# FaspDevTeam/faspsolver

Hardware: AMD Instinct MI355X
Metric: AMG-PCG solve DOF/s (3D 7-pt Poisson 256^3, classical AMG V(1,1) w-Jacobi + PCG, rtol 1e-8) (higher is better)
Workload: dtype f64

## Files before the change

faspsolver_amd/__init__.py:

```python
import ctypes as C
import os
import subprocess

import numpy as np

from . import _types as T
from ._types import *

_HERE = os.path.dirname(os.path.abspath(__file__))
LIB_PATH = os.environ.get("FASP_HIP_LIB") or os.path.join(_HERE, "libfasp_hip.so")
_lib = None

EXPORTS = [
    "fasp_param_amg_init", "fasp_param_solver_init", "fasp_solver_dcsr_krylov_amg",
    "fasp_blas_dcsr_mxv", "fasp_blas_dcsr_aAxpy", "fasp_blas_darray_dotprod",
    "fasp_blas_darray_norm2", "fasp_blas_darray_norminf", "fasp_blas_darray_axpy",
    "fasp_blas_darray_axpby", "fasp_smoother_dcsr_jacobi",
    "fasp_blas_dbsr_mxv", "fasp_blas_dbsr_aAxpy", "fasp_dbsr_getdiaginv", "fasp_smoother_dbsr_jacobi1",
    "fasp_solver_dbsr_pcg", "fasp_solver_dbsr_pbcgs", "fasp_solver_dbsr_pgmres", "fasp_solver_dbsr_pvgmres",
    "fasp_solver_dbsr_pvfgmres", "fasp_hip_bsr_precond_setup", "fasp_hip_bsr_precond_fct", "fasp_hip_bsr_precond_free",
    "fasp_hip_param_input", "fasp_fwrapper_dcsr_krylov_amg_", "fasp_dcsrvec_read2", "fasp_dvec_read",
    "fasp_dbsr_read", "fasp_dcoo_read", "fasp_dcoo_read1", "fasp_dcoo_shift_read", "fasp_dmtx_read", "fasp_dmtxsym_read", "fasp_dvec_write", "fasp_dcsr_write_coo", "fasp_dcsrvec_write2", "fasp_fwrapper_dcsr_amg_", "fasp_fwrapper_dbsr_krylov_amg_", "fasp_hip_free_bsr", "fasp_hip_comm_selftest", "fasp_hip_amg_kernel_info", "fasp_hip_coarse_kernel_info", "fasp_hip_bsr_coarse_kernel_info", "fasp_hip_coding_selftest", "fasp_solver_amg", "fasp_solver_famg", "fasp_hip_amg_solve", "fasp_precond_diag", "fasp_precond_dbsr_diag", "fasp_solver_dcsr_itsolver", "fasp_solver_dcsr_krylov", "fasp_solver_dcsr_krylov_diag", "fasp_solver_dbsr_itsolver", "fasp_solver_dbsr_krylov", "fasp_solver_dbsr_krylov_diag", "fasp_hip_mxv_csr", "fasp_hip_mxv_bsr", "fasp_solver_matfree_init", "fasp_solver_pcg", "fasp_solver_pbcgs", "fasp_solver_pgcg", "fasp_solver_pminres", "fasp_solver_pgmres", "fasp_solver_pvgmres", "fasp_solver_pvfgmres", "fasp_solver_itsolver", "fasp_solver_krylov", "fasp_solver_dcsr_pcg", "fasp_solver_dcsr_pminres", "fasp_solver_dcsr_pgcg", "fasp_solver_dcsr_pgcr", "fasp_solver_dcsr_pbcgs", "fasp_solver_dcsr_pgmres", "fasp_solver_dcsr_pvgmres",
    "fasp_solver_dcsr_pvfgmres", "fasp_hip_precond_setup", "fasp_hip_precond_fct", "fasp_hip_precond_free",
    "fasp_hip_time_bsr_mxv", "fasp_solver_dbsr_krylov_amg", "fasp_hip_bsr_amg_create", "fasp_hip_bsr_amg_create_host",
    "fasp_hip_bsr_amg_destroy", "fasp_hip_bsr_amg_num_levels", "fasp_hip_bsr_amg_get_matrix",
    "fasp_hip_bsr_amg_get_diaginv", "fasp_hip_bsr_solve",
    "fasp_hip_set_device", "fasp_hip_device_count", "fasp_hip_device_identity", "fasp_hip_available",
    "fasp_hip_amg_create", "fasp_hip_amg_create_host", "fasp_hip_amg_upload",
    "fasp_hip_amg_destroy", "fasp_hip_amg_num_levels", "fasp_hip_amg_get_matrix",
    "fasp_hip_amg_get_cfmark", "fasp_hip_solve", "fasp_hip_set_rhs", "fasp_hip_set_guess",
    "fasp_hip_solve_resident", "fasp_hip_get_solution", "fasp_hip_device_synchronize",
    "fasp_hip_precond_amg",
    "fasp_hip_poisson7pt", "fasp_hip_aniso27pt", "fasp_hip_free_system", "fasp_hip_time_kernel", "fasp_hip_measure_ceilings", "fasp_hip_amg_publish", "fasp_hip_amg_attach", "fasp_hip_amg_unpublish",
    "fasp_precond_setup", "fasp_precond_amg", "fasp_precond_famg", "fasp_precond_amli", "fasp_precond_namli", "fasp_amg_data_create", "fasp_amg_data_free", "fasp_param_amg_to_prec", "fasp_param_prec_to_amg", "fasp_mem_free", "fasp_mem_calloc", "fasp_dvec_alloc", "fasp_dvec_set", "fasp_dvec_free", "fasp_dvec_create", "fasp_dcsr_create", "fasp_dcsr_free", "fasp_smoother_dcsr_gs", "fasp_smoother_dcsr_sor", "fasp_smoother_dcsr_L1diag",
    "fasp_hip_tune", "fasp_hip_comm_unique_id", "fasp_hip_comm_init", "fasp_hip_comm_finalize",
    "fasp_hip_comm_rank", "fasp_hip_comm_size", "fasp_hip_version", "fasp_hip_comm_init_shm",
    "fasp_hip_dist_plan", "fasp_hip_dist_level_info", "fasp_hip_dist_get_matrix",
    "fasp_hip_dist_get_list",
    "fasp_blas_dcsr_vmv", "fasp_blas_dcsr_mxv_agg", "fasp_blas_dcsr_aAxpy_agg", "fasp_blas_darray_ax",
    "fasp_blas_darray_axpyz", "fasp_blas_darray_norm1", "fasp_darray_cp", "fasp_darray_set", "fasp_dvec_isnan",
    "fasp_hip_time_matrix", "fasp_hip_bsr_dist_info", "fasp_hip_seq_schedule_selftest", "fasp_hip_seq_chain_selftest", "fasp_hip_cluster_order", "fasp_hip_permute_csr", "fasp_hip_comm_init_ipc", "fasp_hip_comm_stats", "fasp_hip_comm_timing", "fasp_hip_estream_selftest", "fasp_hip_sell_selftest", "fasp_hip_csr_plan", "fasp_hip_level_op", "fasp_hip_matrix_op",
    "fasp_param_ilu_init", "fasp_ilu_data_create", "fasp_ilu_data_free", "fasp_mem_iludata_check", "fasp_ilu_dcsr_setup",
    "fasp_precond_ilu", "fasp_precond_ilu_forward", "fasp_precond_ilu_backward", "fasp_solver_dcsr_krylov_ilu",
    "fasp_solver_dcsr_krylov_ilu_M", "fasp_smoother_dcsr_ilu", "fasp_fwrapper_dcsr_krylov_ilu_",
    "fasp_hip_ilu_resident_count", "fasp_hip_ilu_time",
    "fasp_ilu_dbsr_setup", "fasp_precond_dbsr_ilu", "fasp_solver_dbsr_krylov_ilu", "fasp_smoother_dbsr_ilu",
    "fasp_fwrapper_dbsr_krylov_ilu_",
    "fasp_hip_bsr_amg_get_ilu", "fasp_hip_bsr_amg_ilu_info", "fasp_hip_bsr_amg_ilu_smooth_time",
    "fasp_hip_bsr_sweep",
    "fasp_blas_dcsr_rap", "fasp_hip_dcsr_rap", "fasp_hip_rap_info", "fasp_hip_rap_device_count", "fasp_hip_rap_time",
]


def build(verbose=False):
    cmd = ["make", "-C", os.path.join(_HERE, "csrc")]
    if not verbose:
        cmd.insert(1, "-s")
    subprocess.run(cmd, check=True)


def lib():
    global _lib
    if _lib is not None:
        return _lib
    if not os.path.exists(LIB_PATH):
        build()
    L = C.CDLL(LIB_PATH)
    P = C.POINTER
    L.fasp_param_amg_init.argtypes = [P(T.AMG_param)]
    L.fasp_param_solver_init.argtypes = [P(T.ITS_param)]
    L.fasp_solver_dcsr_krylov_amg.argtypes = [P(T.dCSRmat), P(T.dvector), P(T.dvector),
                                              P(T.ITS_param), P(T.AMG_param)]
    L.fasp_blas_dcsr_mxv.argtypes = [P(T.dCSRmat), T.c_double_p, T.c_double_p]
    L.fasp_blas_dcsr_aAxpy.argtypes = [C.c_double, P(T.dCSRmat), T.c_double_p, T.c_double_p]
    for f in ("fasp_blas_darray_dotprod", "fasp_blas_darray_norm2", "fasp_blas_darray_norminf"):
        getattr(L, f).restype = C.c_double
    L.fasp_blas_darray_dotprod.argtypes = [C.c_int, T.c_double_p, T.c_double_p]
    L.fasp_blas_darray_norm2.argtypes = [C.c_int, T.c_double_p]
    L.fasp_blas_darray_norminf.argtypes = [C.c_int, T.c_double_p]
    L.fasp_blas_darray_axpy.argtypes = [C.c_int, C.c_double, T.c_double_p, T.c_double_p]
    L.fasp_blas_darray_axpby.argtypes = [C.c_int, C.c_double, T.c_double_p, C.c_double,
                                         T.c_double_p]
    L.fasp_blas_dcsr_vmv.restype = C.c_double
    L.fasp_blas_dcsr_vmv.argtypes = [P(T.dCSRmat), T.c_double_p, T.c_double_p]
    L.fasp_blas_dcsr_mxv_agg.argtypes = [P(T.dCSRmat), T.c_double_p, T.c_double_p]
    L.fasp_blas_dcsr_aAxpy_agg.argtypes = [C.c_double, P(T.dCSRmat), T.c_double_p, T.c_double_p]
    L.fasp_blas_darray_ax.argtypes = [C.c_int, C.c_double, T.c_double_p]
    L.fasp_blas_darray_axpyz.argtypes = [C.c_int, C.c_double, T.c_double_p, T.c_double_p, T.c_double_p]
    L.fasp_blas_darray_norm1.restype = C.c_double
    L.fasp_blas_darray_norm1.argtypes = [C.c_int, T.c_double_p]
    L.fasp_darray_cp.argtypes = [C.c_int, T.c_double_p, T.c_double_p]
    L.fasp_darray_set.argtypes = [C.c_int, T.c_double_p, C.c_double]
    L.fasp_hip_time_matrix.restype = C.c_double
    L.fasp_hip_time_matrix.argtypes = [P(T.dCSRmat), C.c_int, C.c_int, P(C.c_int)]
    L.fasp_dvec_isnan.restype = C.c_short
    L.fasp_dvec_isnan.argtypes = [P(T.dvector)]
    L.fasp_smoother_dcsr_jacobi.argtypes = [P(T.dvector), C.c_int, C.c_int, C.c_int,
                                            P(T.dCSRmat), P(T.dvector), C.c_int, C.c_double]
    L.fasp_blas_dbsr_mxv.argtypes = [P(T.dBSRmat), T.c_double_p, T.c_double_p]
    L.fasp_blas_dbsr_aAxpy.argtypes = [C.c_double, P(T.dBSRmat), T.c_double_p, T.c_double_p]
    L.fasp_dbsr_getdiaginv.argtypes = [P(T.dBSRmat)]
    L.fasp_dbsr_getdiaginv.restype = T.dvector
    L.fasp_smoother_dbsr_jacobi1.argtypes = [P(T.dBSRmat), P(T.dvector), P(T.dvector), T.c_double_p]
    L.fasp_hip_bsr_sweep.argtypes = [P(T.dBSRmat), T.c_double_p, T.c_double_p, T.c_double_p, C.c_int, C.c_int, C.c_double,
                                     P(C.c_int)]
    L.fasp_hip_time_bsr_mxv.argtypes = [P(T.dBSRmat), C.c_int]
    L.fasp_hip_time_bsr_mxv.restype = C.c_double
    L.fasp_solver_dcsr_pcg.argtypes = [P(T.dCSRmat), P(T.dvector), P(T.dvector), P(T.precond), C.c_double,
                                       C.c_double, C.c_int, C.c_short, C.c_short]
    L.fasp_solver_dcsr_pbcgs.argtypes = L.fasp_solver_dcsr_pcg.argtypes
    L.fasp_solver_dcsr_pminres.argtypes = L.fasp_solver_dcsr_pcg.argtypes
    L.fasp_solver_dcsr_pgcg.argtypes = L.fasp_solver_dcsr_pcg.argtypes
    L.fasp_solver_dcsr_pvgmres.argtypes = [P(T.dCSRmat), P(T.dvector), P(T.dvector), P(T.precond), C.c_double,
                                           C.c_double, C.c_int, C.c_short, C.c_short, C.c_short]
    L.fasp_solver_dcsr_pvfgmres.argtypes = L.fasp_solver_dcsr_pvgmres.argtypes
    L.fasp_solver_dcsr_pgmres.argtypes = L.fasp_solver_dcsr_pvgmres.argtypes
    L.fasp_solver_dcsr_pgcr.argtypes = L.fasp_solver_dcsr_pvgmres.argtypes
    L.fasp_hip_precond_setup.argtypes = [P(T.dCSRmat), P(T.AMG_param)]
    L.fasp_hip_precond_setup.restype = P(T.precond)
    L.fasp_hip_precond_free.argtypes = [P(T.precond)]
    L.fasp_hip_precond_free.restype = None
    L.fasp_hip_precond_fct.argtypes = [T.c_double_p, T.c_double_p, C.c_void_p]
    L.fasp_hip_precond_fct.restype = None
    L.fasp_solver_dbsr_pcg.argtypes = [P(T.dBSRmat), P(T.dvector), P(T.dvector), P(T.precond), C.c_double,
                                       C.c_double, C.c_int, C.c_short, C.c_short]
    L.fasp_solver_dbsr_pbcgs.argtypes = L.fasp_solver_dbsr_pcg.argtypes
    L.fasp_solver_dbsr_pvgmres.argtypes = [P(T.dBSRmat), P(T.dvector), P(T.dvector), P(T.precond), C.c_double,
                                           C.c_double, C.c_int, C.c_short, C.c_short, C.c_short]
    L.fasp_solver_dbsr_pgmres.argtypes = L.fasp_solver_dbsr_pvgmres.argtypes
    L.fasp_solver_dbsr_pvfgmres.argtypes = L.fasp_solver_dbsr_pvgmres.argtypes
    L.fasp_hip_bsr_precond_setup.argtypes = [P(T.dBSRmat), P(T.AMG_param)]
    L.fasp_hip_bsr_precond_setup.restype = P(T.precond)
    L.fasp_hip_bsr_precond_free.argtypes = [P(T.precond)]
    L.fasp_hip_bsr_precond_free.restype = None
    L.fasp_hip_bsr_precond_fct.argtypes = [T.c_double_p, T.c_double_p, C.c_void_p]
    L.fasp_hip_bsr_precond_fct.restype = None
    L.fasp_dcsrvec_read2.argtypes = [C.c_char_p, C.c_char_p, P(T.dCSRmat), P(T.dvector)]
    L.fasp_dvec_read.argtypes = [C.c_char_p, P(T.dvector)]
    L.fasp_dbsr_read.argtypes = [C.c_char_p, P(T.dBSRmat)]
    L.fasp_hip_free_bsr.argtypes = [P(T.dBSRmat)]
    L.fasp_hip_free_bsr.restype = None
    L.fasp_hip_param_input.argtypes = [C.c_char_p, P(T.ITS_param), P(T.AMG_param)]
    L.fasp_fwrapper_dcsr_krylov_amg_.argtypes = [P(C.c_int), P(C.c_int), T.c_int_p, T.c_int_p, T.c_double_p,
                                                 T.c_double_p, T.c_double_p, P(C.c_double), P(C.c_int), P(C.c_int)]
    L.fasp_fwrapper_dcsr_krylov_amg_.restype = None
    L.fasp_hip_coding_selftest.argtypes = [P(T.dCSRmat), P(C.c_int)]
    L.fasp_hip_amg_kernel_info.argtypes = [C.c_void_p, C.c_int, C.c_int, P(C.c_int), P(C.c_double)]
    L.fasp_hip_coarse_kernel_info.argtypes = [C.c_void_p, P(C.c_int)]
    L.fasp_hip_bsr_coarse_kernel_info.argtypes = [C.c_void_p, P(C.c_int)]
    L.fasp_solver_amg.argtypes = [P(T.dCSRmat), P(T.dvector), P(T.dvector), P(T.AMG_param)]
    L.fasp_hip_amg_solve.argtypes = [C.c_void_p, P(T.dvector), P(T.dvector), P(T.AMG_param), T.c_double_p,
                                     C.c_int, P(T.fasp_hip_stats)]
    L.fasp_solver_dbsr_krylov_amg.argtypes = [P(T.dBSRmat), P(T.dvector), P(T.dvector), P(T.ITS_param),
                                              P(T.AMG_param)]
    L.fasp_hip_bsr_amg_create.argtypes = [P(C.c_void_p), P(T.dBSRmat), P(T.AMG_param)]
    L.fasp_hip_bsr_amg_create_host.argtypes = [P(C.c_void_p), P(T.dBSRmat), P(T.AMG_param)]
    L.fasp_hip_bsr_amg_destroy.argtypes = [C.c_void_p]
    L.fasp_hip_bsr_amg_destroy.restype = None
    L.fasp_hip_bsr_amg_num_levels.argtypes = [C.c_void_p]
    L.fasp_hip_bsr_amg_get_matrix.argtypes = [C.c_void_p, C.c_int, C.c_int, P(T.dBSRmat)]
    L.fasp_hip_bsr_amg_get_diaginv.argtypes = [C.c_void_p, C.c_int]
    L.fasp_hip_bsr_amg_get_diaginv.restype = T.c_double_p
    L.fasp_hip_bsr_solve.argtypes = [C.c_void_p, P(T.dvector), P(T.dvector), P(T.ITS_param), T.c_double_p,
                                     C.c_int, P(T.fasp_hip_stats)]
    L.fasp_hip_amg_create.argtypes = [P(C.c_void_p), P(T.dCSRmat), P(T.AMG_param)]
    L.fasp_hip_amg_create_host.argtypes = L.fasp_hip_amg_create.argtypes
    L.fasp_hip_amg_upload.argtypes = [C.c_void_p]
    L.fasp_hip_amg_destroy.argtypes = [C.c_void_p]
    L.fasp_hip_amg_destroy.restype = None
    L.fasp_hip_amg_num_levels.argtypes = [C.c_void_p]
    L.fasp_hip_amg_get_matrix.argtypes = [C.c_void_p, C.c_int, C.c_int, P(T.dCSRmat)]
    L.fasp_hip_amg_get_cfmark.argtypes = [C.c_void_p, C.c_int, P(T.ivector)]
    L.fasp_hip_solve.argtypes = [C.c_void_p, P(T.dvector), P(T.dvector), P(T.ITS_param),
                                 T.c_double_p, C.c_int, P(T.fasp_hip_stats)]
    L.fasp_hip_set_rhs.argtypes = [C.c_void_p, P(T.dvector)]
# ... 471 lines not shown
```

faspsolver_amd/csrc/coarse_cg.hip.h:

```cpp

static bool small_coarse_ok(long long rows, long long stored_values)
{
    static int enabled = -1;
    if (enabled < 0) {
        const char* e = std::getenv("FASP_HIP_SMALL_COARSE");
        enabled = (e && std::atoi(e) == 0) ? 0 : 1;
    }
    return enabled && rows <= 4096 && stored_values <= 131072;
}
static SmallOut* small_out_dev() { return reinterpret_cast<SmallOut*>(g_ctx.d_partials2); }
static int small_out_fetch(SmallOut& o)
{
    HIPCK(hipMemcpyAsync(g_ctx.h_part, g_ctx.d_partials2, sizeof(SmallOut), hipMemcpyDeviceToHost, g_ctx.stream));
    HIPCK(hipStreamSynchronize(g_ctx.stream));
    std::memcpy(&o, g_ctx.h_part, sizeof(SmallOut));
    return 0;
}

static bool g_persist_disabled = false;
static bool build_persist_plan(fasp_hip_amg* h, int level)
{
    auto& P = h->persist;
    if (P.tried) return P.ok;
    P.tried = true;
    const HostCSR& A = h->H.L[(size_t)level].A;
    const int m = A.row;
    const int nblocks = g_ctx.num_cu, nw = (nblocks - 1) * 8;
    if (m < 1 || m > 6144 || m != A.col || nw < 8 || A.nnz <= 0) return false;
    std::vector<int> order((size_t)m), slots((size_t)m);
    for (int i = 0; i < m; ++i) { order[(size_t)i] = i; slots[(size_t)i] = (A.ia[i + 1] - A.ia[i] + 63) / 64; }
    std::stable_sort(order.begin(), order.end(), [&](int x, int y) { return slots[(size_t)x] > slots[(size_t)y]; });
    std::vector<int> load((size_t)nw, 0), cnt((size_t)nw, 0), wrow((size_t)nw * 8, -1), wend((size_t)nw * 8, 0);
    std::vector<std::pair<int, int>> heap;
    for (int w = 0; w < nw; ++w) heap.emplace_back(0, w);
    auto cmp = [](const std::pair<int, int>& x, const std::pair<int, int>& y) { return x > y; };
    std::make_heap(heap.begin(), heap.end(), cmp);
    for (int i : order) {
        if (slots[(size_t)i] == 0) continue;
        std::pop_heap(heap.begin(), heap.end(), cmp);
        std::pair<int, int> top = heap.back();
        const int w = top.second;
        if (cnt[(size_t)w] >= 8) return false;
        load[(size_t)w] += slots[(size_t)i];
        wrow[(size_t)w * 8 + cnt[(size_t)w]] = i;
        wend[(size_t)w * 8 + cnt[(size_t)w]] = load[(size_t)w];
        cnt[(size_t)w]++;
        heap.back() = std::make_pair(load[(size_t)w], w);
        std::push_heap(heap.begin(), heap.end(), cmp);
    }
    for (int i = 0; i < m; ++i) if (slots[(size_t)i] == 0) return false;
    const int maxload = *std::max_element(load.begin(), load.end());
    const int NE = maxload <= 32 ? 32 : maxload <= 48 ? 48 : maxload <= 56 ? 56 : maxload <= 64 ? 64 : 0;
    if (!NE) return false;
    const size_t tot = (size_t)nw * NE * 64;
    Buf<double> vals(tot);
    Buf<unsigned short> cols(tot);
    std::memset(vals.data(), 0, tot * sizeof(double));
    std::memset(cols.data(), 0, tot * sizeof(unsigned short));
#pragma omp parallel for schedule(dynamic, 16)
    for (int w = 0; w < nw; ++w) {
        int base = 0;
        for (int j = 0; j < cnt[(size_t)w]; ++j) {
            const int row = wrow[(size_t)w * 8 + j];
            const int kb = A.ia[row], len = A.ia[row + 1] - kb;
            for (int e = 0; e < len; ++e) {
                const size_t at = ((size_t)w * NE + base + e / 64) * 64 + (size_t)(e % 64);
                vals[at] = A.val[kb + e];
                cols[at] = (unsigned short)(A.ja[kb + e] * 8);
            }
            base = wend[(size_t)w * 8 + j];
        }
    }
    bool ok = hipMalloc(&P.vals, tot * sizeof(double)) == hipSuccess && hipMalloc(&P.cols, tot * sizeof(unsigned short)) == hipSuccess &&
              hipMalloc(&P.wrow, sizeof(int) * (size_t)nw * 8) == hipSuccess && hipMalloc(&P.wend, sizeof(int) * (size_t)nw * 8) == hipSuccess &&
              hipMalloc(&P.t2, sizeof(double) * 4 * (size_t)m) == hipSuccess && hipMalloc(&P.sync, 1024) == hipSuccess;
    if (ok) ok = hipMemcpy(P.vals, vals.data(), tot * sizeof(double), hipMemcpyHostToDevice) == hipSuccess &&
                 hipMemcpy(P.cols, cols.data(), tot * sizeof(unsigned short), hipMemcpyHostToDevice) == hipSuccess &&
                 hipMemcpy(P.wrow, wrow.data(), sizeof(int) * (size_t)nw * 8, hipMemcpyHostToDevice) == hipSuccess &&
                 hipMemcpy(P.wend, wend.data(), sizeof(int) * (size_t)nw * 8, hipMemcpyHostToDevice) == hipSuccess;
    if (ok) ok = hipMemset(P.t2, 0, sizeof(double) * 4 * (size_t)m) == hipSuccess;
    if (!ok) return false;
    P.NE = NE; P.nblocks = nblocks; P.ok = true;
    return true;
}

template <int NE>
static int launch_spcg_persist(const SpcgPersistArgs& pa, size_t lds)
{
    static bool attr = false;
    if (!attr) {
        HIPCK(hipFuncSetAttribute((const void*)k_spcg_persist<NE>, hipFuncAttributeMaxDynamicSharedMemorySize, 160 * 1024 - 1024));
        attr = true;
    }
    hipLaunchKernelGGL(k_spcg_persist<NE>, dim3(pa.nblocks - (g_tune.spcg_test_hang ? 1 : 0)), dim3(512), lds, g_ctx.stream, pa);
    return FASP_SUCCESS;
}

static int coarse_spcg(fasp_hip_amg* h, DevLevel& D, double tol, int prtlvl)
{
    const DevCSR& A = D.A;
    const int m = A.row;
    const int nn = (int)((unsigned)m * (unsigned)m);
    const int MaxIt = std::max(250, std::min(nn, 1000));
    if (small_coarse_ok(m, A.nnz)) {
        SpcgArgs a{};
        a.A = SmallCSR{m, A.ia, A.ja, A.val};
        a.b = D.b; a.u = D.x; a.p = h->cp; a.r = h->cr; a.t = h->ct; a.u_best = h->cbest;
        a.tol = tol; a.MaxIt = MaxIt; a.x_zero = D.x_zero ? 1 : 0; a.out = small_out_dev(); a.nnz = A.nnz;
        a.lazy = h->lazy_active ? h->d_lazy : nullptr;
        const size_t lds_v = sizeof(double) * 5 * (size_t)m;
        const size_t lds_m = 12 * (size_t)A.nnz + 4 * ((size_t)m + 1);
        static bool attr = false;
        if (!attr) {
            (void)hipFuncSetAttribute((const void*)k_spcg_small<true, true>, hipFuncAttributeMaxDynamicSharedMemorySize, 150 * 1024);
            (void)hipFuncSetAttribute((const void*)k_spcg_small<true, false>, hipFuncAttributeMaxDynamicSharedMemorySize, 150 * 1024);
            attr = true;
        }
        int LD = m; while (LD % 32 != 1) ++LD;
        const size_t lds_w = sizeof(double) * (128 * (size_t)LD + 128);
        const bool one_wave = g_tune.small_onewave && m <= 128 && lds_w <= 148 * 1024;
        if (one_wave && g_tune.small_onewave >= 3) {
            const int NBK = m <= 64 ? 4 : m <= 96 ? 6 : 8, DUP = NBK == 4 ? 4 : 2, RB = NBK / DUP;
            if (!h->reg_img || h->reg_mc != -NBK) {
                const HostCSR& Ah = h->H.L.back().A;
                const int NT = 16 * NBK * DUP;
                std::vector<double> img((size_t)RB * 16 * NT, 0.0);
                for (int row = 0; row < m; ++row)
                    for (int k = Ah.ia[row]; k < Ah.ia[row + 1]; ++k) {
                        const int c = Ah.ja[k], cb = c >> 4, j = c & 15, rb = row >> 4, l = row & 15;
                        const int half = rb / RB, kk = rb % RB, g = half * NBK + cb;
                        img[(size_t)(kk * 16 + j) * NT + 16 * g + l] += Ah.val[k];
                    }
                if (h->reg_img) (void)hipFree(h->reg_img);
                HIPCK(hipMalloc((void**)&h->reg_img, sizeof(double) * img.size()));
                HIPCK(hipMemcpy(h->reg_img, img.data(), sizeof(double) * img.size(), hipMemcpyHostToDevice));
                h->reg_mc = -NBK;
            }
            a.img = h->reg_img;
            const bool ahead = g_tune.small_onewave >= 4;
            h->coarse_kinfo[0] = 1; h->coarse_kinfo[1] = NBK; h->coarse_kinfo[2] = ahead ? 1 : 0;
            if (NBK == 4 && ahead) hipLaunchKernelGGL((k_spcg_dpp<4, 4, true>), dim3(1), dim3(320), 0, g_ctx.stream, a, LD);
            else if (NBK == 4) hipLaunchKernelGGL((k_spcg_dpp<4, 4, false>), dim3(1), dim3(256), 0, g_ctx.stream, a, LD);
            else if (NBK == 6 && ahead) hipLaunchKernelGGL((k_spcg_dpp<6, 2, true>), dim3(1), dim3(256), 0, g_ctx.stream, a, LD);
            else if (NBK == 6) hipLaunchKernelGGL((k_spcg_dpp<6, 2, false>), dim3(1), dim3(192), 0, g_ctx.stream, a, LD);
            else if (ahead) hipLaunchKernelGGL((k_spcg_dpp<8, 2, true>), dim3(1), dim3(320), 0, g_ctx.stream, a, LD);
            else hipLaunchKernelGGL((k_spcg_dpp<8, 2, false>), dim3(1), dim3(256), 0, g_ctx.stream, a, LD);
        }
        else if (one_wave && g_tune.small_onewave >= 2) {
            const int MC = m <= 64 ? 32 : m <= 96 ? 48 : 64;
            if (!h->reg_img || h->reg_mc != MC) {
                const HostCSR& Ah = h->H.L.back().A;
                std::vector<double> img((size_t)MC * SPCG_REG_NT, 0.0);
                for (int row = 0; row < m; ++row)
                    for (int k = Ah.ia[row]; k < Ah.ia[row + 1]; ++k) {
                        const int c = Ah.ja[k], hh = (c >> 1) & 1, kk = 2 * (c >> 2) + (c & 1);
                        if (kk < MC) img[(size_t)kk * SPCG_REG_NT + 2 * row + hh] += Ah.val[k];
                    }
                if (h->reg_img) (void)hipFree(h->reg_img);
                HIPCK(hipMalloc((void**)&h->reg_img, sizeof(double) * img.size()));
                HIPCK(hipMemcpy(h->reg_img, img.data(), sizeof(double) * img.size(), hipMemcpyHostToDevice));
                h->reg_mc = MC;
            }
            a.img = h->reg_img;
            static bool attr_r = false;
            if (!attr_r) {
                (void)hipFuncSetAttribute((const void*)k_spcg_reg<32>, hipFuncAttributeMaxDynamicSharedMemorySize, 150 * 1024);
                (void)hipFuncSetAttribute((const void*)k_spcg_reg<48>, hipFuncAttributeMaxDynamicSharedMemorySize, 150 * 1024);
                (void)hipFuncSetAttribute((const void*)k_spcg_reg<64>, hipFuncAttributeMaxDynamicSharedMemorySize, 150 * 1024);
                attr_r = true;
            }
            const size_t lds_r = sizeof(double) * (2 * (size_t)MC + 4);
            h->coarse_kinfo[0] = 2; h->coarse_kinfo[1] = MC; h->coarse_kinfo[2] = 0;
            if (m <= 64) hipLaunchKernelGGL(k_spcg_reg<32>, dim3(1), dim3(SPCG_REG_NT), lds_r, g_ctx.stream, a, LD);
            else if (m <= 96) hipLaunchKernelGGL(k_spcg_reg<48>, dim3(1), dim3(SPCG_REG_NT), lds_r, g_ctx.stream, a, LD);
            else hipLaunchKernelGGL(k_spcg_reg<64>, dim3(1), dim3(SPCG_REG_NT), lds_r, g_ctx.stream, a, LD);
        }
        else if (one_wave) {
            static bool attr_w = false;
            if (!attr_w) { (void)hipFuncSetAttribute((const void*)k_spcg_wave, hipFuncAttributeMaxDynamicSharedMemorySize, 150 * 1024); attr_w = true; }
            hipLaunchKernelGGL(k_spcg_wave, dim3(1), dim3(64), lds_w, g_ctx.stream, a, LD);
            h->coarse_kinfo[0] = 3; h->coarse_kinfo[1] = 0; h->coarse_kinfo[2] = 0;
        }
        else if (g_tune.small_lds && lds_v + lds_m <= 148 * 1024) {
            hipLaunchKernelGGL((k_spcg_small<true, true>), dim3(1), dim3(SMALL_BLOCK), lds_v + lds_m, g_ctx.stream, a);
            h->coarse_kinfo[0] = 4; h->coarse_kinfo[1] = 2; h->coarse_kinfo[2] = 0;
        }
        else if (g_tune.small_lds && lds_v <= 148 * 1024) {
            hipLaunchKernelGGL((k_spcg_small<true, false>), dim3(1), dim3(SMALL_BLOCK), lds_v, g_ctx.stream, a);
            h->coarse_kinfo[0] = 4; h->coarse_kinfo[1] = 1; h->coarse_kinfo[2] = 0;
        }
        else {
            hipLaunchKernelGGL((k_spcg_small<false, false>), dim3(1), dim3(SMALL_BLOCK), 0, g_ctx.stream, a);
            h->coarse_kinfo[0] = 4; h->coarse_kinfo[1] = 0; h->coarse_kinfo[2] = 0;
        }
        D.x_zero = false;
        if (a.lazy) return FASP_SUCCESS;
        SmallOut o;
        if (small_out_fetch(o) < 0) return ERROR_MISC;
        h->coarse_iters += o.iters;
        if (std::getenv("FASP_HIP_DEBUG_COARSE")) std::printf("[coarse small] status %d iters %d relres %.6e\n", o.status, o.iters, o.relres);
        return o.status;
    }
    const double maxdiff = tol * STAG_RATIO;
    int iter = 0, stag = 1, more_step = 1, iter_best = 0;
    double absres0 = BIGREAL, absres = BIGREAL, relres = BIGREAL, normu = BIGREAL, normr0 = BIGREAL;
    double reldiff, factor, alpha = 0.0, beta, temp1, temp2, absres_best = BIGREAL;
    double *p = h->cp, *r = h->cr, *t = h->ct, *u_best = h->cbest, *u = D.x;
    const double* b = D.b;
    double red[8];
    hipStream_t s = g_ctx.stream;
    (void)prtlvl;

    const bool fused = g_tune.spcg_fused && m <= 8000 && A.val && A.ja && !A.code && !A.pat;
    bool persist = fused && g_tune.spcg_persist && !g_persist_disabled && !comm_shares_devices() &&
                   (size_t)m * 24 <= 150 * 1024 && build_persist_plan(h, (int)(&D - &h->L[0]));
    if (!h->spcg_state) HIPCK(hipMalloc(&h->spcg_state, sizeof(SpcgState)));
    if (fused) {
        if (!D.x_zero) d_resid(A, u, b, r);
        SpcgInitArgs ia{};
        ia.m = m; ia.x_zero = D.x_zero ? 1 : 0; ia.MaxIt = MaxIt; ia.tol = tol; ia.maxdiff = maxdiff;
        ia.b = b; ia.u = u; ia.r = r; ia.p = p; ia.u_best = u_best; ia.st = h->spcg_state;
        hipLaunchKernelGGL(k_spcg_init, dim3(1), dim3(512), 0, s, ia);
        D.x_zero = false;
        goto ITERATE;
    }

    HIPCK(hipMemsetAsync(u_best, 0, sizeof(double) * m, s));

    if (D.x_zero) {
        HIPCK(hipMemcpyAsync(r, b, sizeof(double) * m, hipMemcpyDeviceToDevice, s));
        HIPCK(hipMemsetAsync(u, 0, sizeof(double) * m, s));
        D.x_zero = false;
    } else {
        d_resid(A, u, b, r);
    }
    if (d_dot(m, r, r, red) < 0) return ERROR_MISC;
    absres0 = std::sqrt(red[0]);
    normr0  = std::max(SMALLREAL, absres0);
    relres  = absres0 / normr0;
    if (relres < tol) goto FINISHED;
    HIPCK(hipMemcpyAsync(p, r, sizeof(double) * m, hipMemcpyDeviceToDevice, s));
    temp1 = red[0];

ITERATE:
    {
        int batch = std::max(1, std::min(g_tune.spcg_batch > 0 ? g_tune.spcg_batch : 8, 64));
        const int batch_next = batch;
        if (fused && h->spcg_last_iters > 0) batch = std::max(4, std::min(h->spcg_last_iters + 1, 96));
        SpcgState S{};
        if (!fused) {
            S.temp1 = temp1; S.temp1_prev = temp1; S.absres_best = absres_best; S.normr0 = normr0; S.tol = tol;
            S.maxdiff = maxdiff; S.iter = 0; S.iter_best = 0; S.stag = stag; S.MaxIt = MaxIt; S.stop = SPCG_RUN;
            S.absres = absres; S.relres = relres; S.alpha = 0.0;
            HIPCK(hipMemcpyAsync(h->spcg_state, &S, sizeof(S), hipMemcpyHostToDevice, s));
        }
        double *R[2] = {r, nullptr}, *P[2] = {p, nullptr}, *T[2] = {t, nullptr};
        SpcgBc* bc = nullptr;
        int  cur = 0;
        bool first = true;
        if (fused) {
            if (!h->spcg_fused_buf) HIPCK(hipMalloc(&h->spcg_fused_buf, sizeof(double) * (3 * (size_t)m + 4)));
            R[1] = h->spcg_fused_buf; P[1] = R[1] + m; T[1] = P[1] + m;
            bc = reinterpret_cast<SpcgBc*>(T[1] + m);
        }
        for (;;) {
            if (persist) {
                auto& PP = h->persist;
                PP.launches = (PP.launches + 1u) & 0x1fffffu;
                if (PP.launches == 0u) { HIPCK(hipMemsetAsync(PP.t2, 0, sizeof(double) * 4 * (size_t)m, s)); PP.launches = 1u; }
                SpcgPersistArgs pa{};
                pa.epoch0 = PP.launches << 11;
                pa.m = m; pa.max_steps = MaxIt + 2; pa.nblocks = PP.nblocks; pa.st = h->spcg_state;
                pa.r = r; pa.p = p; pa.u = u; pa.u_best = u_best; pa.t2 = PP.t2; pa.sync = PP.sync;
                pa.vals = PP.vals; pa.cols = PP.cols; pa.wrow = PP.wrow; pa.wend = PP.wend;
                HIPCK(hipMemsetAsync(PP.sync, 0, 1024, s));
                pa.u_lds = (sizeof(double) * 4 * (size_t)m + 1024 <= 160 * 1024) ? 1 : 0;
                const size_t lds = sizeof(double) * (pa.u_lds ? 4 : 3) * (size_t)m;
                int lst;
                if (PP.NE == 32) lst = launch_spcg_persist<32>(pa, lds);
                else if (PP.NE == 48) lst = launch_spcg_persist<48>(pa, lds);
                else if (PP.NE == 56) lst = launch_spcg_persist<56>(pa, lds);
                else lst = launch_spcg_persist<64>(pa, lds);
                if (lst < 0) return lst;
                h->coarse_kinfo[0] = 6; h->coarse_kinfo[1] = PP.NE; h->coarse_kinfo[2] = pa.u_lds;
            }
            for (int q = 0; q < batch && fused && !persist; ++q) {
                SpcgFusedArgs fa{};
                fa.m = m; fa.first = first ? 1 : 0; fa.in = cur; fa.st = h->spcg_state; fa.bc = bc;
                fa.ia = A.ia; fa.ja = A.ja; fa.ja16 = A.jbase ? nullptr : A.ja16; fa.val = A.val;
                for (int k = 0; k < 2; ++k) { fa.r[k] = R[k]; fa.p[k] = P[k]; fa.t[k] = T[k]; }
                fa.u = u; fa.u_best = u_best;
                const int cap = g_tune.spcg_grid > 0 ? g_tune.spcg_grid : 2 * g_ctx.num_cu - 1;
                const dim3 grid(1 + std::max(1, std::min((m + 7) / 8, cap)));
                const size_t lds = sizeof(double) * (size_t)m;
                if (m <= 512 * 4) hipLaunchKernelGGL(k_spcg_fused<4>, grid, dim3(512), lds, s, fa);
                else if (m <= 512 * 10) hipLaunchKernelGGL(k_spcg_fused<10>, grid, dim3(512), lds, s, fa);
                else hipLaunchKernelGGL(k_spcg_fused<16>, grid, dim3(512), lds, s, fa);
                h->coarse_kinfo[0] = 5; h->coarse_kinfo[1] = m <= 512 * 4 ? 4 : m <= 512 * 10 ? 10 : 16; h->coarse_kinfo[2] = 0;
                cur ^= 1; first = false;
            }
            for (int q = 0; q < batch && !fused; ++q) {
                CsrArgs a{}; a.x = p; a.y = t; a.dotv = p; a.partials = g_ctx.d_partials; a.stop = &h->spcg_state->stop;
                SpcgStepArgs sa{};
                sa.m = m; sa.st = h->spcg_state; sa.t = t; sa.p = p; sa.u = u; sa.r = r; sa.u_best = u_best;
                sa.ntp = launch_csr<OP_MXV_DOT>(A, a);
                sa.tp_partials = g_ctx.d_partials;
                if (m <= 512 * 4) hipLaunchKernelGGL(k_spcg_step_reg<4>, dim3(1), dim3(512), 0, s, sa);
                else if (m <= 512 * 10) hipLaunchKernelGGL(k_spcg_step_reg<10>, dim3(1), dim3(512), 0, s, sa);
                else hipLaunchKernelGGL(k_spcg_step, dim3(1), dim3(SMALL_BLOCK), 0, s, sa);
                h->coarse_kinfo[0] = 7; h->coarse_kinfo[1] = m <= 512 * 4 ? 4 : m <= 512 * 10 ? 10 : 0; h->coarse_kinfo[2] = 0;
            }
            bool spec_rr = false;
            if (persist && g_tune.spcg_spec) {
                d_resid(A, u, b, t);
                if (d_dot_to(m, t, t, 14, false) < 0) return ERROR_MISC;
                spec_rr = true;
            }
            HIPCK(hipMemcpyAsync(g_ctx.h_part, h->spcg_state, sizeof(SpcgState), hipMemcpyDeviceToHost, s));
            static_assert(sizeof(SpcgState) % 8 == 0 && sizeof(SpcgState) + 24 <= sizeof(double) * 64, "the error word and the speculative norm travel behind the state");
            if (persist) HIPCK(hipMemcpyAsync(reinterpret_cast<char*>(g_ctx.h_part) + sizeof(SpcgState), h->persist.sync, 16, hipMemcpyDeviceToHost, s));
            if (spec_rr) HIPCK(hipMemcpyAsync(reinterpret_cast<char*>(g_ctx.h_part) + sizeof(SpcgState) + 16, g_ctx.d_red + 14, 8, hipMemcpyDeviceToHost, s));
            HIPCK(hipStreamSynchronize(s));
            std::memcpy(&S, g_ctx.h_part, sizeof(S));
            double spec_val = 0.0;
            if (spec_rr) std::memcpy(&spec_val, reinterpret_cast<char*>(g_ctx.h_part) + sizeof(SpcgState) + 16, 8);
            if (persist) {
                unsigned ew[4];
                std::memcpy(ew, reinterpret_cast<char*>(g_ctx.h_part) + sizeof(SpcgState), 16);
                if (ew[3] != 0u && S.stop == SPCG_RUN) S.stop = SPCG_HANG;
            }
            iter = S.iter; absres_best = S.absres_best; iter_best = S.iter_best;
            batch = batch_next;
            if (fused) {
                normr0 = S.normr0;
                if (S.stop == SPCG_ZERO_RHS) { relres = S.relres; goto FINISHED; }
            }
#ifdef SPCG_PERSIST_STAMPS
            if (persist) {
                unsigned dbg[64];
                (void)hipMemcpy(dbg, h->persist.sync, sizeof(dbg), hipMemcpyDeviceToHost);
                std::printf("[persist stamps, 10 ns ticks, %d steps] lead:", S.iter);
                for (int q = 0; q < 8; ++q) std::printf(" %u", dbg[32 + q]);
                std::printf(" | block 1:");
                for (int q = 0; q < 8; ++q) std::printf(" %u", dbg[40 + q]);
                std::printf("   (spmv meet(second group of records + verdict) read step(tail) pass1-2 pass3 first-group-of-records(block 1) poll-rounds)\n");
            }
#endif
            if (S.stop == SPCG_HANG) {
                std::fprintf(stderr, "### WARNING: fasp_hip: the persistent coarse CG kernel timed out waiting for a block that was not "
                                     "resident (is another process using this GPU?); continuing with the per-iteration kernels\n");
                g_persist_disabled = true;
                persist = false;
                S.stop = SPCG_RUN;
                HIPCK(hipMemcpyAsync(h->spcg_state, &S, sizeof(S), hipMemcpyHostToDevice, s));
                HIPCK(hipStreamSynchronize(s));
                cur = 0; first = true;
                continue;
            }
            if (S.stop == SPCG_RUN) continue;
            if (fused && !persist) { cur = S.pad; r = R[cur]; p = P[cur]; first = true; }
            temp2 = S.tp; temp1 = S.temp1_prev;
            red[0] = S.rr; red[1] = S.uu; red[2] = S.pp; red[3] = S.maxu; red[4] = S.nan;
            alpha = S.alpha; absres = S.absres; relres = S.relres;
            if (S.stop == SPCG_DIV0) goto RESTORE_BESTSOL;
            factor = absres / absres0; (void)factor; (void)alpha;
            if (S.stop == SPCG_NAN) { absres = BIGREAL; goto RESTORE_BESTSOL; }
            if (S.stop == SPCG_SOLSTAG) { iter = ERROR_SOLVER_SOLSTAG; break; }
            if (S.stop == SPCG_MAXIT) { iter = MaxIt + 1; break; }
            normu = std::sqrt(red[1]);
            reldiff = std::fabs(S.alpha) * std::sqrt(red[2]) / normu;
            if ((stag <= MAX_STAG) & (reldiff < maxdiff)) {
                spec_rr = false;
                d_resid(A, u, b, r);
                if (d_dot(m, r, r, red) < 0) return ERROR_MISC;
                absres = std::sqrt(red[0]);
                relres = absres / normr0;
                if (relres < tol) break;
                if (stag >= MAX_STAG) { iter = ERROR_SOLVER_STAG; break; }
                HIPCK(hipMemsetAsync(p, 0, sizeof(double) * m, s));
                ++stag;
            }
            if (relres < tol) {
                if (spec_rr && S.stop != SPCG_HANG) red[0] = spec_val;
                else {
                    spec_rr = false;
                    d_resid(A, u, b, r);
                    if (d_dot(m, r, r, red) < 0) return ERROR_MISC;
                }
                absres = std::sqrt(red[0]);
                relres = absres / normr0;
                if (relres < tol) break;
                if (spec_rr) HIPCK(hipMemcpyAsync(r, t, sizeof(double) * m, hipMemcpyDeviceToDevice, s));
                if (more_step >= MAX_RESTART) { iter = ERROR_SOLVER_TOLSMALL; break; }
                HIPCK(hipMemsetAsync(p, 0, sizeof(double) * m, s));
                ++more_step;
            }
            absres0 = absres;
            temp2 = red[0];
            beta = temp2 / temp1;
            temp1 = temp2;
            d_axpby(m, 1.0, r, beta, p);
            S.temp1 = temp1; S.temp1_prev = temp1; S.stag = stag; S.stop = SPCG_RUN;
            HIPCK(hipMemcpyAsync(h->spcg_state, &S, sizeof(S), hipMemcpyHostToDevice, s));
            HIPCK(hipStreamSynchronize(s));
        }
    }

RESTORE_BESTSOL:
    if (iter != iter_best) {
        d_resid(A, u_best, b, r);
        if (d_dot(m, r, r, red) < 0) return ERROR_MISC;
        absres_best = std::sqrt(red[0]);
        if (absres > absres_best + maxdiff || std::isnan(absres)) {
            HIPCK(hipMemcpyAsync(u, u_best, sizeof(double) * m, hipMemcpyDeviceToDevice, s));
            relres = absres_best / normr0;
        }
    }
FINISHED:
    if (std::getenv("FASP_HIP_DEBUG_COARSE")) std::printf("[coarse batched] iter %d relres %.6e absres %.6e best %d\n", iter, relres, absres, iter_best);
    if (iter > 0) { h->coarse_iters += iter; h->spcg_last_iters = iter; }
    if (iter > MaxIt) return ERROR_SOLVER_MAXIT;
    return iter;
}
```

faspsolver_amd/csrc/device_csr.hip.h:

```cpp

struct DevCSR {
    int     row = 0, col = 0, nnz = 0;
    int*    ia  = nullptr;
    int*    ja  = nullptr;
    double* val = nullptr;
    int*    dpos = nullptr;
    bool    dup_diag = false;
    bool    sorted = false;
    int     lanes = 8;
    int     kind = 0;
    int     tile_rows = 256;
    int     wrows = 64, wcap = 512;
    unsigned char* code = nullptr;
    int*    rowbase = nullptr;
    int*    doff = nullptr;
    double* dval = nullptr;
    unsigned short* pat = nullptr;
    int*    pstart = nullptr;
    int*    plen = nullptr;
    int*    poff = nullptr;
    double* pval = nullptr;
    int     npat = 0, npent = 0;
    unsigned short* ja16 = nullptr;
    int*            jbase = nullptr;
// ... 829 lines not shown
    HIPCK(hipMalloc(&D.sell_tab, sizeof(double) * (size_t)S.nv));
    HIPCK(hipMemcpy(D.sell_code, S.code.data(), sizeof(unsigned) * (size_t)S.slots, hipMemcpyHostToDevice));
    HIPCK(hipMemcpy(D.sell_meta, meta.data(), sizeof(int) * meta.size(), hipMemcpyHostToDevice));
    HIPCK(hipMemcpy(D.sell_rlen, S.rlen.data(), (size_t)H.row, hipMemcpyHostToDevice));
    HIPCK(hipMemcpy(D.sell_tab, S.tab.data(), sizeof(double) * (size_t)S.nv, hipMemcpyHostToDevice));
    D.sell_nv = S.nv; D.sell_obits = S.obits; D.sell_nslice = S.nslice; D.sell_slots = S.slots;
    return FASP_SUCCESS;
}

static int upload_csr(const HostCSR& H, DevCSR& D)
{
    D.row = H.row; D.col = H.col; D.nnz = H.nnz;
    HIPCK(hipMalloc(&D.ia, sizeof(int) * ((size_t)H.row + 1)));
    HIPCK(hipMalloc(&D.ja, sizeof(int) * std::max<size_t>(H.nnz, 1)));
    HIPCK(hipMalloc(&D.val, sizeof(double) * (std::max<size_t>(H.nnz, 1) + 2)));
    HIPCK(hipMemsetAsync(D.val + std::max<size_t>(H.nnz, 1), 0, sizeof(double) * 2, g_ctx.stream));
    HIPCK(hipMemcpyAsync(D.ia, H.ia.data(), sizeof(int) * ((size_t)H.row + 1), hipMemcpyHostToDevice, g_ctx.stream));
    pick_kernel(D);
    auto upload_plain = [&]() -> int {
        HIPCK(hipMemcpyAsync(D.ja, H.ja.data(), sizeof(int) * (size_t)H.nnz, hipMemcpyHostToDevice, g_ctx.stream));
        HIPCK(hipMemcpyAsync(D.val, H.val.data(), sizeof(double) * (size_t)H.nnz, hipMemcpyHostToDevice, g_ctx.stream));
        return 0;
    };
    if (compress_enabled() && H.nnz >= 4096 && (double)H.nnz <= 48.0 * H.row) {
        Buf<unsigned short> pat; Buf<int> prb;
        std::vector<int> pstart, plen, poff; std::vector<double> pval;
        static const bool rowpat_on = !(std::getenv("FASP_HIP_ROWPAT") && std::atoi(std::getenv("FASP_HIP_ROWPAT")) == 0);
        if (rowpat_on && build_rowpat(H, pat, pstart, plen, poff, pval, prb)) {
            D.npat = (int)pstart.size(); D.npent = (int)poff.size();
            HIPCK(hipMalloc(&D.pat, sizeof(unsigned short) * ((size_t)H.row + 2)));
            HIPCK(hipMalloc(&D.pstart, sizeof(int) * pstart.size()));
            HIPCK(hipMalloc(&D.plen, sizeof(int) * plen.size()));
            HIPCK(hipMemcpy(D.plen, plen.data(), sizeof(int) * plen.size(), hipMemcpyHostToDevice));
            HIPCK(hipMalloc(&D.poff, sizeof(int) * std::max<size_t>(poff.size(), 1)));
            HIPCK(hipMalloc(&D.pval, sizeof(double) * std::max<size_t>(pval.size(), 1)));
            HIPCK(hipMemset(D.pat + H.row, 0xff, sizeof(unsigned short) * 2));
            HIPCK(hipMemcpy(D.pat, pat.data(), sizeof(unsigned short) * (size_t)H.row, hipMemcpyHostToDevice));
            HIPCK(hipMemcpy(D.pstart, pstart.data(), sizeof(int) * pstart.size(), hipMemcpyHostToDevice));
            HIPCK(hipMemcpy(D.poff, poff.data(), sizeof(int) * poff.size(), hipMemcpyHostToDevice));
            HIPCK(hipMemcpy(D.pval, pval.data(), sizeof(double) * pval.size(), hipMemcpyHostToDevice));
            if (prb.n) {
                HIPCK(hipMalloc(&D.rowbase, sizeof(int) * ((size_t)H.row + 2)));
                HIPCK(hipMemcpy(D.rowbase, prb.data(), sizeof(int) * (size_t)H.row, hipMemcpyHostToDevice));
                const int nr = H.row, npair = (nr + 1) / 2;
                long long nx = 0;
#pragma omp parallel for schedule(static) reduction(+ : nx)
                for (int w0 = 0; w0 < nr; w0 += 128) {
                    const int    pm = std::min((w0 + 64) / 2, npair - 1);
                    const unsigned domA = pat[(size_t)2 * pm], domB = (2 * pm + 1 < nr) ? pat[(size_t)2 * pm + 1] : 0xffffu;
                    for (int r = w0; r < std::min(w0 + 128, nr); r += 2) {
                        const bool vb = r + 1 < nr;
                        if (!(vb && pat[r] == domA && pat[r + 1] == domB)) nx += vb ? 2 : 1;
                    }
                }
                if (nx * 4 <= nr) D.nxrows = (int)nx;
            } else {
                D.plane = grid_plane_of(poff, H.row);
                if (std::getenv("FASP_HIP_SETUP_TIMING")) std::printf("        [upload_csr %d x %d, %d nnz] %d row patterns; grid plane for the XCD strips: %d rows\n", H.row, H.col, H.nnz, (int)pstart.size(), D.plane);
                const int nr = H.row, npair = (nr + 1) / 2;
                long long nx = 0;
#pragma omp parallel for schedule(static) reduction(+ : nx)
                for (int w0 = 0; w0 < nr; w0 += 128) {
                    const unsigned dom = pat[(size_t)2 * std::min((w0 + 64) / 2, npair - 1)];
                    for (int r = w0; r < std::min(w0 + 128, nr); r += 2) {
                        const bool vb = r + 1 < nr;
                        if (!(vb && pat[r] == dom && pat[r + 1] == dom)) nx += vb ? 2 : 1;
                    }
                }
                if (nx * 4 <= nr) D.nxrows = (int)nx;
            }
            D.kind = 2;
            return upload_plain() < 0 ? ERROR_ALLOC_MEM : FASP_SUCCESS;
        }
        std::vector<int> doff; std::vector<double> dval;
        Buf<unsigned char> code; Buf<int> rowbase;
        if (build_dict8(H, doff, dval, code, rowbase)) {
            HIPCK(hipMalloc(&D.code, (size_t)H.nnz + 256));
            HIPCK(hipMalloc(&D.doff, sizeof(int) * 256));
            HIPCK(hipMalloc(&D.dval, sizeof(double) * 256));
            HIPCK(hipMemcpy(D.code, code.data(), (size_t)H.nnz, hipMemcpyHostToDevice));
            HIPCK(hipMemcpy(D.doff, doff.data(), sizeof(int) * 256, hipMemcpyHostToDevice));
            HIPCK(hipMemcpy(D.dval, dval.data(), sizeof(double) * 256, hipMemcpyHostToDevice));
            if (rowbase.n) {
                HIPCK(hipMalloc(&D.rowbase, sizeof(int) * (size_t)H.row));
                HIPCK(hipMemcpy(D.rowbase, rowbase.data(), sizeof(int) * (size_t)H.row, hipMemcpyHostToDevice));
            }
            D.kind = 2;
            return upload_plain() < 0 ? ERROR_ALLOC_MEM : FASP_SUCCESS;
        }
    }
    static const bool sort_long = !(std::getenv("FASP_HIP_SORT_LONG_ROWS") && std::atoi(std::getenv("FASP_HIP_SORT_LONG_ROWS")) == 0);
    static const int  sort_stream = std::getenv("FASP_HIP_SORT_STREAM") ? std::atoi(std::getenv("FASP_HIP_SORT_STREAM")) : 0;
    const double avg_len = H.row > 0 ? (double)H.nnz / H.row : 0.0;
    const bool do_sort = sort_long && !g_oneshot_upload && H.nnz > 0 && (D.kind == 0 || (D.kind == 2 && sort_stream > 0 && avg_len >= sort_stream));
    static const bool timing = std::getenv("FASP_HIP_SETUP_TIMING") != nullptr;
    double tp = wall_seconds();
    auto lap = [&](const char* what) {
        if (!timing) return;
        const double now = wall_seconds();
        std::printf("        [upload_csr %d x %d, %d nnz] %-10s %8.3f s\n", H.row, H.col, H.nnz, what, now - tp);
        tp = now;
    };
    if (do_sort && D.kind == 0) {
        int maxlen = 0;
#pragma omp parallel for schedule(static) reduction(max : maxlen)
        for (int i = 0; i < H.row; ++i) maxlen = std::max(maxlen, H.ia[i + 1] - H.ia[i]);
        if (g_device_sort && maxlen <= SORT_MAXLEN) {
            const int st = upload_sorted_on_device(H, D, maxlen);
            lap("device sort");
            return st < 0 ? st : build_estream(H.ia.data(), H.row, H.nnz, D);
        }
    }
    if (do_sort) {
        Buf<int> sj((size_t)H.nnz);
        Buf<double> sv((size_t)H.nnz);
        std::vector<int> dp;
        const bool square = H.row == H.col;
        if (square) dp.assign((size_t)H.row, -1);
#pragma omp parallel
        {
            std::vector<std::pair<int, double>> tmp;
#pragma omp for schedule(dynamic, 64)
            for (int i = 0; i < H.row; ++i) {
                const int kb = H.ia[i], ke = H.ia[i + 1];
                tmp.resize((size_t)(ke - kb));
                for (int k = kb; k < ke; ++k) tmp[(size_t)(k - kb)] = {H.ja[k], H.val[k]};
                std::stable_sort(tmp.begin(), tmp.end(),
                                 [](const std::pair<int, double>& x, const std::pair<int, double>& y) { return x.first < y.first; });
                for (int k = kb; k < ke; ++k) {
                    sj[k] = tmp[(size_t)(k - kb)].first; sv[k] = tmp[(size_t)(k - kb)].second;
                    if (square && sj[k] == i) dp[(size_t)i] = k;
                }
            }
        }
        lap("row sort");
        HIPCK(hipMemcpy(D.ja, sj.data(), sizeof(int) * (size_t)H.nnz, hipMemcpyHostToDevice));
        HIPCK(hipMemcpy(D.val, sv.data(), sizeof(double) * (size_t)H.nnz, hipMemcpyHostToDevice));
        lap("memcpy");
        if (square && D.kind == 2) {
            HIPCK(hipMalloc(&D.dpos, sizeof(int) * (size_t)std::max(H.row, 1)));
            HIPCK(hipMemcpy(D.dpos, dp.data(), sizeof(int) * (size_t)H.row, hipMemcpyHostToDevice));
        }
        D.sorted = true;
        if (upload_ja16(D, H.ia.data(), sj.data()) < 0) return ERROR_ALLOC_MEM;
        return build_estream(H.ia.data(), H.row, H.nnz, D);
    }
    if (upload_plain() < 0) return ERROR_ALLOC_MEM;
    if (D.kind == 2 && !g_oneshot_upload && build_xtile(H, D) < 0) return ERROR_ALLOC_MEM;
    if (D.kind == 2 && compress_enabled() && upload_sell(H, D) < 0) return ERROR_ALLOC_MEM;
    if (upload_ja16(D, H.ia.data(), H.ja.data()) < 0) return ERROR_ALLOC_MEM;
    return build_estream(H.ia.data(), H.row, H.nnz, D);
}

struct Tuning { int ilu_smooth_fused = 1, gen2 = 2, ws2_bpc = 3, maxgrid = -1, xcd = 16, nt = 1, kind = -1, lanes = -1, wrows = -1, wcap = -1, compress = 1, rpl = -1, lds_tab = 1, xcd_pat = 64, spcg_batch = 16, small_lds = 1, ja16 = 1, spcg_fused = 1, spcg_grid = 0, spcg_persist = 1, split_rows = 0, gs_multicolor = 0, seq_flow = 1, seq_strip_kb = 0, seq_jobs = 1, seq_spine = 1, seq_grid = 0, seq_chain = 1, seq_chain_n1 = 0, seq_chain_grid = 0, seq_chain_ref = 0, seq_test_hang = 0, seq_rest_lanes = 0, local_square = 1, fuse_zr = 1, fuse_presmooth = 1, seq_lanes = 0, xtile = 1, rp5_max = 45, rp_bpc = 5, rp_xcd = -1, rp_strip = 2, spcg_test_hang = 0, small_onewave = 4, lazy_coarse = 1, rp_stream = -1, renumber = 1, renumber_chunk = 262144, pcg_dev_beta = 1, spcg_spec = 1, ev_every = 4, pcg_fold = 1, seq_chain_touch = 8, seq_chain_touch_t1 = 1, seq_zero_skip = 1, estream = 1, es_dbg = 0, ilu_form = -1, sell = 1; };
static Tuning g_tune;

template <class K>
static int resident_blocks_per_cu(K kernel)
{
    static std::vector<std::pair<const void*, int>> cache;
    const void* key = reinterpret_cast<const void*>(kernel);
    for (const auto& e : cache)
        if (e.first == key) return e.second;
    int nb = 0;
    if (hipOccupancyMaxActiveBlocksPerMultiprocessor(&nb, kernel, BLOCK, 0) != hipSuccess || nb < 1) nb = 4;
    nb = std::min(nb, 8);
    cache.emplace_back(key, nb);
    return nb;
}

template <class K>
static int launch_persistent(K kernel, int ntiles, CsrArgs& a, int blocks_per_cu = 0)
{
    int cap = (blocks_per_cu > 0 ? std::min(blocks_per_cu, resident_blocks_per_cu(kernel)) : resident_blocks_per_cu(kernel)) * g_ctx.num_cu;
    if (g_tune.maxgrid > 0) cap = g_tune.maxgrid;
    cap = std::min(cap, MAXGRID);
    int grid = std::min(cap, ntiles);
    grid = std::max(8, (grid + 7) / 8 * 8);
    hipLaunchKernelGGL(kernel, dim3(grid), dim3(BLOCK), 0, g_ctx.stream, a);
    return grid;
}

enum CsrKernel : int {
    CK_ROWS_2 = 0, CK_ROWS_4, CK_ROWS_8, CK_ROWS_16, CK_ROWS_32, CK_ROWS_64,
    CK_WSTREAM_64_512, CK_WSTREAM_64_1024, CK_WSTREAM_32_512, CK_WSTREAM_32_1024,
    CK_ROWPAT_0_1, CK_ROWPAT_0_2, CK_ROWPAT_1_1, CK_ROWPAT_1_2, CK_ROWPAT_2_1, CK_ROWPAT_2_2,
    CK_DICT8_8, CK_DICT8_16, CK_DICT8_24,
    CK_ESTREAM_4, CK_ESTREAM_8, CK_ESTREAM_16, CK_ESTREAM_32,
    CK_ROWPAT4, CK_ROWPAT5, CK_LSTREAM, CK_XTILE, CK_SELL, CK_WSTREAM2
};
struct CsrPlan {
    CsrKernel kernel;
    int    family;
    int    tile_rows;
    int    bpc;
    int    xcd_map;
    int    tpp;
    int    nt;
    bool   ja16, jbase;
    bool   fused_zr;
    double bytes;
};
static CsrPlan plan_csr(const DevCSR& M, int op, bool windowed, bool want_partials, int rows = -1)
{
    CsrPlan p{};
    int kind = M.kind;
    if (rows < 0) rows = M.row;
    if (M.code && g_tune.compress) kind = 4;
    if (M.pat && g_tune.compress) kind = 5;
    if (g_tune.kind >= 0 && !(g_tune.kind == 4 && !M.code) && !(g_tune.kind == 5 && !M.pat)) kind = g_tune.kind;
    const int lanes = g_tune.lanes > 0 ? g_tune.lanes : M.lanes, wrows = g_tune.wrows > 0 ? g_tune.wrows : M.wrows, wcap = g_tune.wcap > 0 ? g_tune.wcap : M.wcap;
    const bool jac = op == OP_JACOBI, w64 = wrows == 64 && wcap == 512;
    const bool lstream_ok = g_tune.gen2 && kind == 2 && w64 && (double)M.nnz <= 7.6 * M.row;
    if (jac && kind != 0 && kind < 4 && (M.dup_diag || !M.dpos) && !lstream_ok) kind = 0;
    p.xcd_map = g_tune.xcd;
    p.nt = g_tune.nt | ((g_tune.rp_stream > 0 || (g_tune.rp_stream < 0 && (size_t)M.row * 8 > (size_t)96 << 20)) ? 4 : 0);
    p.ja16 = g_tune.ja16 && M.ja16; p.jbase = g_tune.ja16 && M.jbase;
    if (M.jbase && kind != 0) p.ja16 = p.jbase = false;
    if (kind == 1 || kind == 3) kind = 0;
    p.tile_rows = kind >= 4 ? BLOCK : kind == 2 ? 4 * wrows : BLOCK / lanes;
    auto ntiles = [&] { return (rows + p.tile_rows - 1) / p.tile_rows; };
    auto strips = [&] {
        const int rpb = p.tile_rows;
        if (!g_tune.rp_strip || M.plane < 8 * rpb || M.plane % (8 * rpb) != 0 || ntiles() < 4 * (M.plane / rpb)) return;
        p.xcd_map = -2; p.tpp = M.plane / rpb;
    };
    const double avg = M.row > 0 ? (double)M.nnz / M.row : 1.0, ptr_bytes = 4.0 * (M.row + 1.0), base_bytes = M.rowbase ? 4.0 * M.row : 0.0;
    const bool pair = kind == 5 && M.nxrows >= 0 && g_tune.rpl <= 0;
    p.bytes = kind == 5 ? 2.0 * M.row + base_bytes + 12.0 * M.npent : kind == 4 ? 1.0 * M.nnz + ptr_bytes + base_bytes : 12.0 * M.nnz + ptr_bytes;
    if (pair && g_tune.gen2 && !M.rowbase) {
        p.kernel = CK_ROWPAT4; p.family = 6; p.tile_rows = 2 * BLOCK;
        p.xcd_map = ntiles() >= 8 * 64 ? g_tune.rp_xcd : 16;
        if (p.xcd_map == -1) strips();
        p.bpc = p.xcd_map == -2 && g_tune.rp_bpc == 5 ? 3 : g_tune.rp_bpc;
        p.fused_zr = jac && want_partials;
    }
    else if (pair && g_tune.gen2 >= 2 && M.rowbase && !jac && op != OP_L1DIAG && (double)M.nnz <= 0.1 * g_tune.rp5_max * M.row) {
        p.kernel = CK_ROWPAT5; p.family = 9; p.tile_rows = 2 * BLOCK; p.bpc = 5;
        p.xcd_map = ntiles() >= 8 * 64 ? -1 : 16;
        if (g_tune.rp_strip >= 2) strips();
    }
    else if (kind == 5) {
        const int rpl = g_tune.rpl > 0 ? g_tune.rpl : 1;
        const bool lds = M.npat <= 512 && M.npent <= 2048 && g_tune.lds_tab != 0;
        const int T = !lds ? 0 : M.npat <= 64 && M.npent <= 512 && g_tune.lds_tab != 3 ? 2 : 1;
        p.kernel = CsrKernel(CK_ROWPAT_0_1 + 2 * T + (rpl != 1)); p.family = 5; p.tile_rows = BLOCK * rpl;
        if (g_tune.xcd_pat != 0) p.xcd_map = g_tune.xcd_pat;
        if (g_tune.xcd_pat == 64 && g_tune.rp_strip >= 2) strips();
    }
    else if (kind == 4) { p.kernel = avg <= 8.5 ? CK_DICT8_8 : avg <= 20.0 ? CK_DICT8_16 : CK_DICT8_24; p.family = 4; }
    else if (lstream_ok) { p.kernel = CK_LSTREAM; p.family = 7; p.bpc = 4; p.fused_zr = jac && want_partials; }
    else if (kind == 2 && g_tune.gen2 >= 2 && w64) {
        if (g_tune.xtile && M.lja16) {
            p.kernel = CK_XTILE; p.family = 10; p.bpc = 3;
            p.bytes = 10.0 * M.nnz + ptr_bytes + 4.0 * M.ntcols + 4.0 * ((M.row + 63) / 64 + 1.0);
        }
        else if (M.sell_code && g_tune.compress && g_tune.sell) {
            p.kernel = CK_SELL; p.family = 11; p.tile_rows = SELL_BLOCK;
            p.bytes = 4.0 * (double)M.sell_slots + 1.0 * M.row + 4.0 * (2.0 * M.sell_nslice + 1.0) + 8.0 * M.sell_nv;
        }
        else { p.kernel = CK_WSTREAM2; p.family = 8; p.bpc = g_tune.ws2_bpc; }
        p.fused_zr = jac && want_partials;
    }
    else if (kind == 2) {
        p.kernel = w64 ? CK_WSTREAM_64_512 : wrows == 64 ? CK_WSTREAM_64_1024 : wrows == 32 && wcap == 512 ? CK_WSTREAM_32_512 : CK_WSTREAM_32_1024; p.family = 2;
    }
    else {
        if (p.ja16) p.bytes = 10.0 * M.nnz + ptr_bytes + (p.jbase ? 4.0 * M.row : 0.0);
        const bool es_rule = g_tune.estream >= 2 || (g_tune.estream == 1 && (double)M.nnz < 256.0 * M.row);
        if (M.es_tab && es_rule && p.ja16 && !windowed && op != OP_MXV_DOT && !(jac && (want_partials || M.dup_diag)))
            p.kernel = avg >= 512.0 ? CK_ESTREAM_32 : avg >= 256.0 ? CK_ESTREAM_16 : avg >= 128.0 ? CK_ESTREAM_8 : CK_ESTREAM_4;
        else
            p.kernel = lanes == 2 ? CK_ROWS_2 : lanes == 4 ? CK_ROWS_4 : lanes == 8 ? CK_ROWS_8 : lanes == 16 ? CK_ROWS_16 : lanes == 32 ? CK_ROWS_32 : CK_ROWS_64;
    }
    return p;
}
static int kernel_family(const DevCSR& M, double* matrix_bytes)
{
    const CsrPlan p = plan_csr(M, OP_MXV, false, false);
    if (matrix_bytes) *matrix_bytes = p.bytes;
    return p.family;
}

template <int OP>
static int launch_sell(const DevCSR& M, CsrArgs& a)
{
    a.sell_code = M.sell_code; a.sell_sptr = M.sell_meta; a.sell_sbase = M.sell_meta + M.sell_nslice + 1; a.sell_rlen = M.sell_rlen;
    a.sell_tab = M.sell_tab; a.sell_nv = M.sell_nv; a.sell_obits = M.sell_obits;
    const size_t lds = sizeof(double) * ((size_t)M.sell_nv + SELL_NW);
    static bool attr_set = false;
    if (!attr_set) {
        (void)hipFuncSetAttribute(reinterpret_cast<const void*>(k_csr_sell<OP>), hipFuncAttributeMaxDynamicSharedMemorySize, (int)(sizeof(double) * (SELL_MAXV + SELL_NW)));
        attr_set = true;
    }
    static std::vector<std::pair<size_t, int>> cache;
    int nb = 0;
    for (const auto& e : cache)
        if (e.first == lds) nb = e.second;
    if (nb == 0) {
        if (hipOccupancyMaxActiveBlocksPerMultiprocessor(&nb, k_csr_sell<OP>, SELL_BLOCK, lds) != hipSuccess || nb < 1) nb = 1;
        nb = std::min(nb, 2);
        cache.emplace_back(lds, nb);
    }
    int cap = nb * g_ctx.num_cu;
    if (g_tune.maxgrid > 0) cap = g_tune.maxgrid;
    cap = std::min(cap, MAXGRID);
    int grid = std::min(cap, a.ntiles);
// ... 214 lines not shown
```

faspsolver_amd/csrc/hierarchy.hip.h:

```cpp

struct DevLevel {
    DevCSR  A, P, R;
    double* diag = nullptr;
    double* l1   = nullptr;
    double *b = nullptr, *xa = nullptr, *xb = nullptr, *w = nullptr;
    double* x  = nullptr;
    double* xo = nullptr;
    bool    x_zero = true;
    bool    presmoothed = false;
    double* halo_pending = nullptr;
    bool    owns_b = true;
    bool    replicated = true;
    int     nloc = 0;
    int     nvec = 0;
    int     row0 = 0;
    int     nglobal = 0;
    std::vector<int> send_off, recv_off;
    int*    d_send_idx = nullptr;
    double* d_sendbuf  = nullptr;
    bool    has_halo() const { return !replicated && nvec > nloc; }
    struct Sched {
        bool built = false, multicolor = false; int* d_order = nullptr; int* d_ptr = nullptr; std::vector<int> ptr;
        int ns = 0, L = 1, LR = 1, pfmax = 1, kt = 0, par = 1, nstrips = 0, nchunk = 0, maxent = 0; bool nolower = false, flow_ok = false, rowlevels = false, independent = false; int nrows = 0, nvirt = 0, nclasses = 0; long long nghost = 0, slot_bytes = 0;
        std::vector<int> cptr;
        void* d_strips = nullptr; void* d_chunks = nullptr; unsigned char* d_slots = nullptr; int* d_gpos = nullptr; int* d_cstrip = nullptr; int* d_lchunks = nullptr;
        int* d_ria = nullptr; int* d_rja = nullptr; double* d_rval = nullptr; double* d_rec = nullptr; double* d_dr = nullptr; int* d_tr = nullptr; double* d_W = nullptr; unsigned* d_prog = nullptr;
        bool chain = false; int nb = 0, npad = 0, n1b = 0, rx = 0, rg = 0; long long t1_steps = 0, t2_steps = 0, nband = 0, nt1 = 0, nt2 = 0;
        double* d_band = nullptr; double* d_drd = nullptr; void* d_blk = nullptr; double* d_t1v = nullptr; double* d_t2v = nullptr;
        unsigned short* d_t1c = nullptr; unsigned short* d_t2c = nullptr; double* d_G2 = nullptr; int* d_t1need = nullptr; int* d_t2need = nullptr;
        std::vector<void*> owned;
        void release()
        {
            if (!owned.empty()) { for (void* q : owned) (void)hipFree(q); owned.clear(); }
            else { if (d_order) (void)hipFree(d_order); if (d_ptr) (void)hipFree(d_ptr); }
            d_order = nullptr; d_ptr = nullptr; built = false;
        }
    };
    Sched   sched[5];
    struct Poly { bool built = false; double* dinv = nullptr; double k[6] = {0, 0, 0, 0, 0, 0}; double* w[5] = {nullptr, nullptr, nullptr, nullptr, nullptr}; };
    Poly    poly;
    int*    d_perm = nullptr;
    bool    diag_uniform = false;
    double  diag_value = 0.0;
    int*    d_mark = nullptr;
    double* w2 = nullptr;
    double* kw[4] = {nullptr, nullptr, nullptr, nullptr};
};

struct EventPair { hipEvent_t a, b; };

struct HipWsMem {
    static int  alloc(double** q, size_t n) { HIPCK(hipMalloc(q, sizeof(double) * std::max<size_t>(n, 1))); return 0; }
    static int  zero(double* q, size_t n) { HIPCK(hipMemsetAsync(q, 0, sizeof(double) * n, g_ctx.stream)); return 0; }
    static void release(double* q) { (void)hipFree(q); }
};
using KrylovWs = KrylovWsT<HipWsMem>;

}

using namespace fasp;

struct SchedJob { int level = 0, kind = 0, st = 0; bool uploaded = false; SplitHost H; DevLevel::Sched S; std::thread th; };

struct fasp_hip_amg {
    std::vector<std::vector<int>> perm;
    std::vector<std::unique_ptr<SchedJob>> sched_jobs;
    bool                  sched_jobs_started = false;
    std::mutex            sched_mu;
    HostHierarchy         H;
    DistPlan              dist;
    bool                  distributed = false;
    std::vector<DevLevel> L;
    AMG_param             param;
    bool                  want_zr = false;
    bool                  pre_marked = false;
    int                   zr_G = 0;
    double *b = nullptr, *u = nullptr, *p = nullptr, *t = nullptr, *r = nullptr;
    double *cp = nullptr, *cr = nullptr, *ct = nullptr, *cbest = nullptr;
    KrylovWs             gm[2];
    double*              spcg_fused_buf = nullptr;
    int                  spcg_last_iters = 0;
    SpcgState*           spcg_state = nullptr;
    struct Persist { bool tried = false, ok = false; int NE = 0, nblocks = 0; double* vals = nullptr; unsigned short* cols = nullptr;
                     int *wrow = nullptr, *wend = nullptr; double* t2 = nullptr; unsigned* sync = nullptr; unsigned launches = 0; } persist;
    std::vector<double>  amli_coef;
    std::vector<int>     level_cycle_type;
    bool                 use_fmg = false;
    std::vector<EventPair> ev;
    int                    ev_used = 0;
    long long              coarse_iters = 0, vcycles = 0;
    int                    coarse_kinfo[6] = {0, 0, 0, 0, 0, 0};
    int*                   d_lazy = nullptr; int* h_lazy = nullptr; bool lazy_active = false, coarse_sync = false;
    double*                reg_img = nullptr; int reg_mc = 0;
    double                 upload_seconds = 0.0;
};

namespace fasp {

static void free_level(DevLevel& D)
{
    D.A.release(); D.P.release(); D.R.release();
    if (D.diag) (void)hipFree(D.diag);
    if (D.l1) (void)hipFree(D.l1);
    if (D.b && D.owns_b) (void)hipFree(D.b);
    if (D.xa) (void)hipFree(D.xa);
    if (D.xb) (void)hipFree(D.xb);
    if (D.w) (void)hipFree(D.w);
    if (D.d_send_idx) (void)hipFree(D.d_send_idx);
    if (D.d_sendbuf) (void)hipFree(D.d_sendbuf);
    for (auto& sc : D.sched) sc.release();
    if (D.poly.dinv) (void)hipFree(D.poly.dinv);
    for (double* q : D.poly.w) if (q) (void)hipFree(q);
    if (D.d_mark) (void)hipFree(D.d_mark);
    if (D.d_perm) (void)hipFree(D.d_perm);
    D.d_perm = nullptr;
    if (D.w2) (void)hipFree(D.w2);
    for (double* q : D.kw) if (q) (void)hipFree(q);
    D = DevLevel();
}

static int alloc_vec(double** p, size_t n)
{
    HIPCK(hipMalloc(p, sizeof(double) * std::max<size_t>(n, 1)));
    return FASP_SUCCESS;
}

static int upload_diag(const HostCSR& A, DevLevel& D)
{
    const int n = A.row;
    std::vector<double> d(n, 0.0), s(n, 0.0);
    std::vector<int>    dp(n, -1);
    int                 ndup = 0;
#pragma omp parallel for schedule(static) reduction(+ : ndup)
    for (int i = 0; i < n; ++i) {
        double di = 0.0, si = 0.0;
        int    hits = 0;
        for (int k = A.ia[i]; k < A.ia[i + 1]; ++k) {
            if (A.ja[k] == i) { di = A.val[k]; dp[i] = k; ++hits; }
            si += (A.val[k] >= 0.0) ? A.val[k] : -A.val[k];
        }
        d[i] = di; s[i] = si;
        if (hits > 1) ++ndup;
    }
    D.A.dup_diag = ndup > 0;
    {
        bool same = n > 0;
        for (int i = 1; i < n && same; ++i) same = std::memcmp(&d[(size_t)i], &d[0], sizeof(double)) == 0;
        D.diag_uniform = same;
        D.diag_value = same ? d[0] : 0.0;
    }
    if (!D.A.sorted) {
        HIPCK(hipMalloc(&D.A.dpos, sizeof(int) * std::max(n, 1)));
        HIPCK(hipMemcpy(D.A.dpos, dp.data(), sizeof(int) * n, hipMemcpyHostToDevice));
    }
    if (alloc_vec(&D.diag, n) < 0 || alloc_vec(&D.l1, n) < 0) return ERROR_ALLOC_MEM;
    HIPCK(hipMemcpy(D.diag, d.data(), sizeof(double) * n, hipMemcpyHostToDevice));
    HIPCK(hipMemcpy(D.l1, s.data(), sizeof(double) * n, hipMemcpyHostToDevice));
    return FASP_SUCCESS;
}

__global__ __launch_bounds__(BLOCK) void k_pack(int n, const int* __restrict__ idx,
                                                 const double* __restrict__ v, double* __restrict__ out)
{
    for (int i = blockIdx.x * BLOCK + threadIdx.x; i < n; i += gridDim.x * BLOCK) out[i] = v[idx[i]];
}

static int halo_exchange(DevLevel& D, double* v, hipStream_t stream = nullptr)
{
    if (!stream) stream = g_ctx.stream;
    if (D.replicated || comm_size() <= 1 || D.send_off.empty()) return FASP_SUCCESS;
    const int P = comm_size(), me = comm_rank();
    const int nsend = D.send_off.back();
    if (nsend > 0)
        hipLaunchKernelGGL(k_pack, dim3(vec_grid(nsend)), dim3(BLOCK), 0, stream, nsend, D.d_send_idx, v,
                           D.d_sendbuf);
    std::vector<CommXfer> sends, recvs;
    for (int q = 0; q < P; ++q) {
        if (q == me) continue;
        const int ns = D.send_off[q + 1] - D.send_off[q], nr = D.recv_off[q + 1] - D.recv_off[q];
        if (ns > 0) sends.push_back({q, D.d_sendbuf + D.send_off[q], (size_t)ns});
        if (nr > 0) recvs.push_back({q, v + D.nloc + D.recv_off[q], (size_t)nr});
    }
    const int st = comm_exchange(sends.data(), (int)sends.size(), recvs.data(), (int)recvs.size(), stream);
    if (st < 0) comm_mark_failed();
    return st;
}

static int g_seq_partition = std::getenv("FASP_HIP_SEQ_PARTITION") && std::atoi(std::getenv("FASP_HIP_SEQ_PARTITION")) != 0;
static int g_halo_overlap = 1;

static int g_coarse_mode = -1, g_coarse_split_min = 16384;
static bool coarse_split_active(const DevCSR& M)
{
    return (g_coarse_mode == 1 || (g_coarse_mode < 0 && comm_is_peer_window())) && comm_size() > 1 && M.row >= g_coarse_split_min;
}
template <int OP>
static int rep_launch(const DevCSR& M, CsrArgs a)
{
    if (!coarse_split_active(M) || a.partials || a.zx) return launch_csr<OP>(M, a);
    const int P = comm_size(), me = comm_rank();
    const int nwin = (M.row + WIN_ALIGN - 1) / WIN_ALIGN, per = (nwin + P - 1) / P;
    std::vector<int> counts((size_t)P), displs((size_t)P);
    for (int q = 0; q < P; ++q) {
        const int lo = std::min(M.row, q * per * WIN_ALIGN), hi = std::min(M.row, (q + 1) * per * WIN_ALIGN);
        displs[(size_t)q] = lo; counts[(size_t)q] = hi - lo;
    }
    RowWin w; w.lo = displs[(size_t)me]; w.hi = w.lo + counts[(size_t)me]; w.goff = 0;
    int G = 0;
    if (w.hi > w.lo) G = launch_csr<OP>(M, a, w);
    if (comm_allgatherv(a.y + w.lo, counts[(size_t)me], a.y, counts.data(), displs.data(), g_ctx.stream) < 0) { comm_mark_failed(); return -1; }
    return G;
}

template <int OP>
static int dist_launch(DevLevel& V, const DevCSR& M, CsrArgs a, const DevLevel* Out = nullptr)
{
    double* v = const_cast<double*>(a.x);
    if (V.replicated && (!Out || Out->replicated) && comm_size() > 1) return rep_launch<OP>(M, a);
    if (V.replicated || comm_size() <= 1 || V.send_off.empty()) return launch_csr<OP>(M, a);
    if (!g_halo_overlap || M.win_hi < 0) {
        if (halo_exchange(V, v) < 0) return -1;
        return launch_csr<OP>(M, a);
    }
    bool local_ok = hipEventRecord(g_ctx.ev_ready, g_ctx.stream) == hipSuccess &&
                    hipStreamWaitEvent(g_ctx.comm_stream, g_ctx.ev_ready, 0) == hipSuccess;
    if (!local_ok) {
        comm_mark_failed();
        (void)hipStreamSynchronize(g_ctx.stream);
        (void)halo_exchange(V, v);
        (void)launch_csr<OP>(M, a);
        return -1;
    }
    RowWin w;
    w.lo = M.win_lo; w.hi = M.win_hi; w.goff = 0;
    int G = launch_csr<OP>(M, a, w);
// ... 216 lines not shown
```

faspsolver_amd/csrc/small_solvers.hip.h:

```cpp
#pragma once

#include <hip/hip_runtime.h>

namespace fasp {

constexpr int SMALL_BLOCK = 512;
constexpr int SMALL_WAVES = SMALL_BLOCK / 64;
constexpr int SMALL_MAX_RESTART = 32;
constexpr int GM_NE = 16;

struct SmallOut {
    int    status;
    int    iters;
    double relres, absres;
};

__device__ __forceinline__ double dpp_mov_f64(double x, const int ctrl, const int row_mask)
{
    const long long b = __double_as_longlong(x);
    int lo = (int)(b & 0xffffffffll), hi = (int)(b >> 32);
    switch (ctrl) {
        case 0x111: lo = __builtin_amdgcn_update_dpp(0, lo, 0x111, 0xf, 0xf, true); hi = __builtin_amdgcn_update_dpp(0, hi, 0x111, 0xf, 0xf, true); break;
        case 0x112: lo = __builtin_amdgcn_update_dpp(0, lo, 0x112, 0xf, 0xf, true); hi = __builtin_amdgcn_update_dpp(0, hi, 0x112, 0xf, 0xf, true); break;
        case 0x114: lo = __builtin_amdgcn_update_dpp(0, lo, 0x114, 0xf, 0xf, true); hi = __builtin_amdgcn_update_dpp(0, hi, 0x114, 0xf, 0xf, true); break;
// ... 1600 lines not shown
                        lo = __builtin_amdgcn_update_dpp(0, lo, 0x138, 0xf, 0xf, true);
                        hi = __builtin_amdgcn_update_dpp(0, hi, 0x138, 0xf, 0xf, true);
                        return __longlong_as_double(((long long)hi << 32) | (long long)(unsigned)lo);
                    };
                    const double rprev = rs[i - 1];
                    const double bj = g_c * hl;
                    const double ns = -g_s;
                    double cur = hl;
                    for (int st = 1; st < i; ++st) {
                        const double nc = ns * shr1(cur) + bj;
                        cur = (tid >= 1) ? nc : cur;
                    }
                    const double np = g_s * hl + g_c * shr1(cur);
                    const double curL = rdl(cur, i - 1);
                    double g = t * t;
                    g += curL * curL;
                    double gamma = sqrt(g);
                    if (gamma == 0.0) gamma = epsmac;
                    const double ci = curL / gamma, si = t / gamma;
                    const double rsi = -si * rprev, rsp = ci * rprev;
                    const double hfin = si * t + ci * curL;
                    g_c = (tid == i) ? ci : g_c;
                    g_s = (tid == i) ? si : g_s;
                    if (tid >= 1 && tid < i) hh[(tid - 1) * R + (i - 1)] = np;
                    if (tid == 0) {
                        hh[(i - 1) * R + (i - 1)] = hfin; hh[i * R + (i - 1)] = t;
                        c[i - 1] = ci; sn[i - 1] = si; rs[i] = rsi; rs[i - 1] = rsp; sc_rnorm = fabs(rsi);
                    }
                }
            } else {
            for (int j = 0; j < i; ++j) {
                const double* pj = P(j);
                double hv[1] = {0.0};
                for (int e = tid; e < n; e += SMALL_BLOCK) hv[0] += pj[e] * pi[e];
                blk_reduce1<1>(hv, sh2, par);
                const double h = hv[0];
                if (tid == 0) hh[j * R + (i - 1)] = h;
                for (int e = tid; e < n; e += SMALL_BLOCK) pi[e] += -h * pj[e];
            }
            {
                double tv[1] = {0.0};
                for (int e = tid; e < n; e += SMALL_BLOCK) tv[0] += pi[e] * pi[e];
                blk_reduce1<1>(tv, sh2, par);
                t = sqrt(tv[0]);
            }
            if (t != 0.0) {
                const double s = 1.0 / t;
                for (int e = tid; e < n; e += SMALL_BLOCK) pi[e] *= s;
            }
            }
            if (!(n <= 64 * GM_NE)) GMT(2);
            if (!(n <= 64 * GM_NE) && tid == 0) {
                hh[i * R + (i - 1)] = t;
                for (int j = 1; j < i; ++j) {
                    const double tt = hh[(j - 1) * R + (i - 1)];
                    hh[(j - 1) * R + (i - 1)] = sn[j - 1] * hh[j * R + (i - 1)] + c[j - 1] * tt;
                    hh[j * R + (i - 1)] = -sn[j - 1] * tt + c[j - 1] * hh[j * R + (i - 1)];
                }
                double g = hh[i * R + (i - 1)] * hh[i * R + (i - 1)];
                g += hh[(i - 1) * R + (i - 1)] * hh[(i - 1) * R + (i - 1)];
                double gamma = sqrt(g);
                if (gamma == 0.0) gamma = epsmac;
                c[i - 1] = hh[(i - 1) * R + (i - 1)] / gamma;
                sn[i - 1] = hh[i * R + (i - 1)] / gamma;
                rs[i] = -sn[i - 1] * rs[i - 1];
                rs[i - 1] = c[i - 1] * rs[i - 1];
                hh[(i - 1) * R + (i - 1)] = sn[i - 1] * hh[i * R + (i - 1)] + c[i - 1] * hh[(i - 1) * R + (i - 1)];
                sc_rnorm = fabs(rs[i]);
            }
            GMT(3);
            __syncthreads();
            GMT(4);
            absres = r_norm = sc_rnorm;
            relres = absres / absres0;
            if (relres < tol) break;
        }

        if (tid == 0) {
            rs[i - 1] = rs[i - 1] / hh[(i - 1) * R + (i - 1)];
            for (int k = i - 2; k >= 0; k--) {
                double tt = 0.0;
                int j = k + 1;
                for (; j + 5 < i; j += 6) {
                    double hv[6], rv[6];
#pragma unroll
                    for (int e = 0; e < 6; ++e) { hv[e] = hh[k * R + j + e]; rv[e] = rs[j + e]; }
#pragma unroll
                    for (int e = 0; e < 6; ++e) tt -= hv[e] * rv[e];
                }
                for (; j < i; j++) tt -= hh[k * R + j] * rs[j];
                tt += rs[k];
                rs[k] = tt / hh[k * R + k];
            }
        }
        __syncthreads();
        for (int e = tid; e < n; e += SMALL_BLOCK) {
            double we = P(i - 1)[e] * rs[i - 1];
            for (int j = i - 2; j >= 0; j--) we += rs[j] * P(j)[e];
            w[e] = we;
            x[e] += we;
        }
        __syncthreads();

        if (relres < tol) {
            g_resid(x, b, w);
            r_norm = sqrt(blk_dot(n, w, w, sh));
            absres = r_norm;
            relres = absres / absres0;
            if (relres < tol) break;
            for (int e = tid; e < n; e += SMALL_BLOCK) P(0)[e] = w[e];
            i = 0;
        }

        if (tid == 0)
            for (int j = i; j > 0; j--) {
                rs[j - 1] = -sn[j - 1] * rs[j];
                rs[j] = c[j - 1] * rs[j];
            }
        __syncthreads();
        if (i) {
            double* pi = P(i);
            double* p0 = P(0);
            for (int e = tid; e < n; e += SMALL_BLOCK) {
                double v = pi[e];
                v = v + (rs[i] - 1.0) * v;
                for (int j = i - 1; j > 0; j--) v += rs[j] * P(j)[e];
                pi[e] = v;
                double q = p0[e];
                q = q + (rs[0] - 1.0) * q;
                p0[e] = q + v;
            }
        }
        __syncthreads();
        cr = r_norm / r_norm_old;
    }

FINISHED:
#ifdef GM_TIMING
    if (tid == 0 && iter > 20) printf("[gmres_small] iters %d: other %.2f spmv %.2f (wavefront 0: rows < 512 %.2f, rows >= 512 %.2f, barrier %.2f) mgs %.2f givens %.2f barrier %.2f us per iteration\n", iter, gmt[0] * 0.01 / iter, (gmt[1] + gmt[5] + gmt[6]) * 0.01 / iter, gmt[5] * 0.01 / iter, gmt[6] * 0.01 / iter, gmt[1] * 0.01 / iter, gmt[2] * 0.01 / iter, gmt[3] * 0.01 / iter, gmt[4] * 0.01 / iter);
#endif
    if (tid == 0) {
        a.out->iters = iter;
        a.out->status = iter >= MaxIt ? -48 : iter;
        a.out->relres = relres;
        a.out->absres = absres;
    }
}

constexpr int SPCG_HANG = 8;
#ifndef SPCG_POLL_GROUP
#define SPCG_POLL_GROUP 6
#endif

struct SpcgPersistArgs {
    int        m, max_steps, nblocks;
    int        u_lds;
    SpcgState* st;
    double    *r, *p, *u, *u_best;
    double*    t2;
    unsigned*  sync;
    unsigned   epoch0;
    const double*         vals;
    const unsigned short* cols;
    const int*            wrow;
    const int*            wend;
};

__device__ __forceinline__ void lds_barrier()
{
    asm volatile("s_waitcnt lgkmcnt(0)\n\ts_barrier" ::: "memory");
}
template <int NQ, int NW>
__device__ __forceinline__ void blk_reduce_dpp(double (&v)[NQ], double* sh, unsigned maxmask = 0u)
{
    const int lane = threadIdx.x & 63, w = threadIdx.x >> 6;
#pragma unroll
    for (int q = 0; q < NQ; ++q) {
        const bool mx = (maxmask >> q) & 1u;
        const double x = mx ? wave_max_to_lane63(v[q]) : wave_sum_to_lane63(v[q]);
        if (lane == 63) sh[w * NQ + q] = x;
    }
    lds_barrier();
#pragma unroll
    for (int q = 0; q < NQ; ++q) {
        const bool mx = (maxmask >> q) & 1u;
        double x = sh[q];
        for (int k = 1; k < NW; ++k) {
            const double y = sh[k * NQ + q];
            x = mx ? fmax(x, y) : x + y;
        }
        v[q] = x;
    }
    lds_barrier();
}

__device__ __forceinline__ bool absres_improves(double rr, double best, double maxdiff) { return sqrt(rr) < best - maxdiff; }

template <int NE, bool LEAD>
__device__ __forceinline__ void spcg_persist_body(const SpcgPersistArgs& a)
{
    constexpr int NT = 512, NW = 8, E = 12, CH = 6;
    extern __shared__ __attribute__((aligned(16))) double dyn[];
    __shared__ double sh[NW * 4];
    __shared__ int    s_flag;
    typedef __attribute__((address_space(1))) unsigned           gu32;
    typedef __attribute__((address_space(1))) unsigned long long gu64;
    const int tid = threadIdx.x, lane = tid & 63, m = a.m;
    const int wave = __builtin_amdgcn_readfirstlane(tid >> 6);
    constexpr bool lead = LEAD;
    double* sp = dyn;
    double* sr = dyn + m;
    double* st = dyn + 2 * m;
    double* su = dyn + 3 * m;
    gu32* g_err = (gu32*)(a.sync + 3);
    gu64* g_verdict = (gu64*)(a.sync + 8);
    __shared__ int s_hang;
    typedef unsigned int pu32x4 __attribute__((ext_vector_type(4)));
    SpcgState& S = *a.st;
    if (S.stop != SPCG_RUN) return;

    double   v[NE];
    unsigned cpk[NE / 2];
    int      my_rows = 0, endsv = 0, rowsv = -1;
    if (!lead) {
        const int gw = ((int)blockIdx.x - 1) * NW + wave;
        const double* pv = a.vals + ((size_t)gw * NE) * 64 + lane;
        const unsigned short* pc = a.cols + ((size_t)gw * NE) * 64 + lane;
#pragma unroll
        for (int k = 0; k < NE; ++k) v[k] = __builtin_nontemporal_load(pv + (size_t)k * 64);
#pragma unroll
        for (int k = 0; k < NE / 2; ++k)
            cpk[k] = (unsigned)__builtin_nontemporal_load(pc + (size_t)(2 * k) * 64) |
                     ((unsigned)__builtin_nontemporal_load(pc + (size_t)(2 * k + 1) * 64) << 16);
        if (lane < 8) { endsv = a.wend[gw * 8 + lane]; rowsv = a.wrow[gw * 8 + lane]; }
        my_rows = __popcll(__ballot(lane < 8 && rowsv >= 0));
    }
    for (int i = tid; i < m; i += NT) { sp[i] = a.p[i]; sr[i] = a.r[i]; }
    const bool u_lds = a.u_lds != 0;
    if (lead && u_lds) for (int i = tid; i < m; i += NT) su[i] = a.u[i];
    double temp1 = S.temp1;
    const double absres_best0 = S.absres_best, normr0 = S.normr0, tol = S.tol, maxdiff = S.maxdiff;
    const int    it0 = S.iter, stag = S.stag, MaxIt = S.MaxIt;
    double best = absres_best0;
    int    iter_best = S.iter_best;
    double o_tp = S.tp, o_rr = S.rr, o_uu = S.uu, o_pp = S.pp, o_maxu = S.maxu, o_nan = S.nan, o_alpha = S.alpha,
           o_absres = S.absres, o_relres = S.relres, o_temp1_prev = S.temp1_prev;
    int steps_done = 0, my_stop = SPCG_RUN;
    if (tid == 0) {
        s_hang = 0;
        if (lead)
            __hip_atomic_store(g_verdict, ((unsigned long long)(a.epoch0 + 1u) << 32) | (unsigned)SPCG_RUN, __ATOMIC_RELAXED, __HIP_MEMORY_SCOPE_AGENT);
    }
    __syncthreads();
#ifdef SPCG_PERSIST_STAMPS
    unsigned long long tk[8] = {0, 0, 0, 0, 0, 0, 0, 0}, tl = __builtin_amdgcn_s_memrealtime();
#define STAMP(q) do { const unsigned long long tn_ = __builtin_amdgcn_s_memrealtime(); tk[q] += tn_ - tl; tl = tn_; } while (0)
#else
#define STAMP(q) do { } while (0)
#endif

    for (int step = 0; step < a.max_steps; ++step) {
        const int par = step & 1;
        const unsigned ep = a.epoch0 + (unsigned)step + 1u;
        const __amdgpu_buffer_rsrc_t tr =
            __builtin_amdgcn_make_buffer_rsrc(a.t2 + (size_t)par * 2 * m, 0, (int)((unsigned)m * 16u), 0x00020000);
        if (!lead && my_rows > 0 && my_stop == SPCG_RUN) {
            double acc = 0.0;
            int    j = 0;
            int    next_end = __builtin_amdgcn_readlane(endsv, 0);
#pragma unroll
            for (int k = 0; k < NE; ++k) {
                const unsigned off = (k & 1) ? (cpk[k >> 1] >> 16) : (cpk[k >> 1] & 0xffffu);
                const double x = *reinterpret_cast<const double*>(reinterpret_cast<const char*>(sp) + off);
                acc += v[k] * x;
                if ((k & 7) == 7) __builtin_amdgcn_sched_barrier(0);
                if (k + 1 == next_end) {
                    const double ssum = wave_sum_to_lane63(acc);
                    const int row = __builtin_amdgcn_readlane(rowsv, j);
                    if (lane == 63) {
                        const unsigned long long bits = (unsigned long long)__double_as_longlong(ssum);
                        const pu32x4 rec = {(unsigned)bits, ep, (unsigned)(bits >> 32), ep};
                        __builtin_amdgcn_raw_buffer_store_b128(rec, tr, row * 16, 0, 16 );
                    }
                    acc = 0.0;
                    ++j;
                    next_end = (j < 8) ? __builtin_amdgcn_readlane(endsv, j & 7) : -1;
                    if (j >= my_rows) next_end = -1;
                }
            }
        }
        STAMP(0);
        {
            const unsigned long long t0 = __builtin_amdgcn_s_memrealtime();
            bool hung = false;
            unsigned long long vr0 = 0ull;
            if (tid == 0) vr0 = __hip_atomic_load(g_verdict + par, __ATOMIC_RELAXED, __HIP_MEMORY_SCOPE_AGENT);
#pragma unroll 1
            for (int e0 = 0; e0 < E && !hung; e0 += SPCG_POLL_GROUP) {
#ifdef SPCG_PERSIST_STAMPS
                if (e0 == 6 && !LEAD) STAMP(6);
#endif
                unsigned pend = 0u;
#pragma unroll
                for (int e = 0; e < SPCG_POLL_GROUP; ++e) if (tid + (e0 + e) * NT < m) pend |= 1u << e;
                while (pend) {
#ifdef SPCG_PERSIST_STAMPS
                    tk[7] += 1;
#endif
                    pu32x4 q[SPCG_POLL_GROUP];
#pragma unroll
                    for (int e = 0; e < SPCG_POLL_GROUP; ++e)
                        q[e] = __builtin_amdgcn_raw_buffer_load_b128(tr, ((pend >> e) & 1u) ? (tid + (e0 + e) * NT) * 16 : (int)0xfffffff0u, 0, 16 );
#pragma unroll
                    for (int e = 0; e < SPCG_POLL_GROUP; ++e)
                        if (((pend >> e) & 1u) && q[e].y == ep && q[e].w == ep) {
                            st[tid + (e0 + e) * NT] = __longlong_as_double((long long)(((unsigned long long)q[e].z << 32) | q[e].x));
                            pend &= ~(1u << e);
                        }
                    if (pend && __builtin_amdgcn_s_memrealtime() - t0 > 200000000ull) { hung = true; break; }
                }
            }
            if (tid == 0 && !hung) {
                int flag = -1;
                for (bool first = true;; first = false) {
                    const unsigned long long vr = first ? vr0 : __hip_atomic_load(g_verdict + par, __ATOMIC_RELAXED, __HIP_MEMORY_SCOPE_AGENT);
                    if ((unsigned)(vr >> 32) == ep) { flag = (int)(unsigned)vr; break; }
                    __builtin_amdgcn_s_sleep(1);
                    if (__builtin_amdgcn_s_memrealtime() - t0 > 200000000ull) { hung = true; break; }
                }
                s_flag = flag;
            }
            if (hung) {
                s_hang = 1;
                __hip_atomic_store(g_err, 1u, __ATOMIC_RELAXED, __HIP_MEMORY_SCOPE_AGENT);
            }
        }
        lds_barrier();
        STAMP(1);
        if (s_hang) { my_stop = SPCG_HANG; break; }
        const int flag = s_flag;
        if (flag != SPCG_RUN) break;
        if (my_stop != SPCG_RUN) break;
        STAMP(2);
        double v1[1] = {0.0};
#pragma unroll 1
        for (int e0 = 0; e0 < E; e0 += CH) {
            double tv[CH], pv[CH];
#pragma unroll
            for (int e = 0; e < CH; ++e) { const int i = min(tid + (e0 + e) * NT, m - 1); tv[e] = st[i]; pv[e] = sp[i]; }
#pragma unroll
            for (int e = 0; e < CH; ++e) if (tid + (e0 + e) * NT < m) v1[0] += tv[e] * pv[e];
        }
        blk_reduce_dpp<1, NW>(v1, sh);
        const double tp = v1[0];
        if (!(fabs(tp) > 1e-40)) {
            o_tp = tp; steps_done = step + 1; my_stop = SPCG_DIV0;
            break;
        }
        const double alpha = temp1 / tp;
        double red[3] = {0.0, 0.0, 0.0};
#pragma unroll 1
        for (int e0 = 0; e0 < E; e0 += CH) {
            double tv[CH], rv[CH], pv[CH], uv[CH];
#pragma unroll
            for (int e = 0; e < CH; ++e) {
                const int i = min(tid + (e0 + e) * NT, m - 1);
                tv[e] = st[i]; rv[e] = sr[i];
                pv[e] = lead ? sp[i] : 0.0;
                uv[e] = lead ? (u_lds ? su[i] : a.u[i]) : 0.0;
            }
#pragma unroll
            for (int e = 0; e < CH; ++e) {
                const int i = tid + (e0 + e) * NT;
                if (i < m) {
                    const double rn = rv[e] - alpha * tv[e];
                    sr[i] = rn;
                    red[0] += rn * rn;
                    if (lead) {
                        const double ui = uv[e] + alpha * pv[e];
                        if (u_lds) su[i] = ui; else a.u[i] = ui;
                        red[1] += ui * ui; red[2] += pv[e] * pv[e];
                    }
                }
            }
        }
        double maxu = 1.0, nan_u = 0.0;
        if (lead) {
            blk_reduce_dpp<3, NW>(red, sh);
            nan_u = (red[1] != red[1]) ? 1.0 : 0.0;
            if (!(red[1] > 2.0 * m * 1e-40)) {
                double mx[1] = {0.0};
                for (int i = tid; i < m; i += NT) mx[0] = fmax(mx[0], fabs(u_lds ? su[i] : a.u[i]));
                blk_reduce_dpp<1, NW>(mx, sh, 1u);
                maxu = mx[0];
            }
        } else {
            double r1[1] = {red[0]};
            blk_reduce_dpp<1, NW>(r1, sh);
            red[0] = r1[0];
        }
        const double rr = red[0], beta = rr / temp1;
        STAMP(4);
        const bool keep_best = lead && absres_improves(rr, best, maxdiff);
        if (lead) {
            const int it = it0 + step + 1;
            STAMP(6);
            const double sq = sqrt(lane == 0 ? rr : lane == 1 ? red[1] : red[2]);
            auto bc = [&](double x, int from) -> double {
                const unsigned long long bb = (unsigned long long)__double_as_longlong(x);
                const unsigned lo = (unsigned)__builtin_amdgcn_readlane((int)(unsigned)bb, from);
                const unsigned hi = (unsigned)__builtin_amdgcn_readlane((int)(unsigned)(bb >> 32), from);
                return __longlong_as_double((long long)(((unsigned long long)hi << 32) | lo));
            };
            const double absres = bc(sq, 0), normu = bc(sq, 1), sq_pp = bc(sq, 2);
            const double fac = fabs(alpha) * sq_pp;
            const double qd = (lane == 0 ? absres : fac) / (lane == 0 ? normr0 : normu);
            const double relres = bc(qd, 0), reldiff = bc(qd, 1);
            int stop = SPCG_RUN;
            if (nan_u > 0.0) stop = SPCG_NAN;
            else {
                if (absres < best - maxdiff) { best = absres; iter_best = it; }
                if (maxu <= 1e-20) stop = SPCG_SOLSTAG;
                else if ((stag <= 20) & (reldiff < maxdiff)) stop = SPCG_STAG;
                else if (relres < tol) stop = SPCG_CONV;
                if (stop == SPCG_RUN && it >= MaxIt) stop = SPCG_MAXIT;
            }
            o_tp = tp; o_rr = rr; o_uu = red[1]; o_pp = red[2]; o_maxu = maxu; o_nan = nan_u;
            o_alpha = alpha; o_absres = absres; o_relres = relres; o_temp1_prev = temp1;
            my_stop = stop;
            if (tid == 0)
                __hip_atomic_store(g_verdict + (par ^ 1), ((unsigned long long)(ep + 1u) << 32) | (unsigned)stop, __ATOMIC_RELAXED,
                                   __HIP_MEMORY_SCOPE_AGENT);
        }
#pragma unroll 1
        for (int e0 = 0; e0 < E; e0 += CH) {
            double rv[CH], pv[CH];
#pragma unroll
            for (int e = 0; e < CH; ++e) {
                const int i = min(tid + (e0 + e) * NT, m - 1);
                rv[e] = sr[i]; pv[e] = sp[i];
            }
#pragma unroll
            for (int e = 0; e < CH; ++e) {
                const int i = tid + (e0 + e) * NT;
                if (i < m) {
                    sp[i] = 1.0 * rv[e] + beta * pv[e];
                    if (keep_best) a.u_best[i] = u_lds ? su[i] : a.u[i];
                }
            }
        }
        STAMP(5);
        temp1 = rr;
        steps_done = step + 1;
        lds_barrier();
        STAMP(3);
    }
#ifdef SPCG_PERSIST_STAMPS
    if (tid == 0 && blockIdx.x < 2)
        for (int q = 0; q < 8; ++q) a.sync[32 + blockIdx.x * 8 + q] = (unsigned)tk[q];
#endif
#undef STAMP

    if (lead) {
        for (int i = tid; i < m; i += NT) { a.r[i] = sr[i]; a.p[i] = sp[i]; if (u_lds) a.u[i] = su[i]; }
        if (tid == 0) {
            S.tp = o_tp; S.rr = o_rr; S.uu = o_uu; S.pp = o_pp; S.maxu = o_maxu; S.nan = o_nan;
            S.alpha = o_alpha; S.absres = o_absres; S.relres = o_relres;
            S.absres_best = best; S.iter_best = iter_best; S.iter = it0 + steps_done;
            S.temp1_prev = o_temp1_prev;
            S.temp1 = (my_stop == SPCG_DIV0) ? S.temp1 : temp1;
            S.stop = my_stop;
        }
    }
}

template <int NE>
__global__ __launch_bounds__(512) void k_spcg_persist(SpcgPersistArgs a)
{
    if (blockIdx.x == 0) spcg_persist_body<NE, true>(a);
    else spcg_persist_body<NE, false>(a);
}

}
```

faspsolver_amd/csrc/solver.hip:

```cpp
#include <hip/hip_runtime.h>

#include <fcntl.h>
#include <omp.h>
#include <sys/mman.h>
#include <sys/stat.h>
#include <unistd.h>

#include <algorithm>
#include <cfloat>
#include <cmath>
#include <cstdio>
#include <cstdlib>
#include <cstring>
#include <functional>
#include <condition_variable>
#include <memory>
#include <mutex>
#include <string>
#include <thread>
#include <vector>

#include "fasp_comm.h"
#include "fasp_internal.h"
#include "krylov_ws.h"
// ... 359 lines not shown
    double tp = wall_seconds();
    auto lap = [&](const char* what) {
        if (!timing) return;
        const double now = wall_seconds();
        std::printf("  [create] %-28s %8.3f s\n", what, now - tp);
        tp = now;
    };
    static const bool ahead_on = !(std::getenv("FASP_HIP_UPLOAD_AHEAD") && std::atoi(std::getenv("FASP_HIP_UPLOAD_AHEAD")) == 0);
    const bool ahead = ahead_on && comm_size() == 1 && amgparam->AMG_type != SA_AMG && amgparam->AMG_type != UA_AMG &&
                       A->nnz >= 1000000;
    if (ahead) {
        h = new fasp_hip_amg();
        h->param = *amgparam;
        h->L.resize(MAX_AMG_LVL + 1);
        AheadUpload up;
        up.h = h;
        up.th = std::thread([&up] { up.run(); });
        g_on_level_ready = &AheadUpload::on_ready; g_on_level_matrix = &AheadUpload::on_matrix; g_on_level_ready_ctx = &up;
        st = host_setup_rs(A, amgparam, h->H);
        g_on_level_ready = nullptr; g_on_level_matrix = nullptr; g_on_level_ready_ctx = nullptr;
        lap("host setup");
        if (st >= 0) {
            { std::lock_guard<std::mutex> lk(up.mu); up.coarsest = (int)h->H.L.size() - 1; }
            AheadUpload::on_ready((int)h->H.L.size() - 1, &up);
        }
        { std::lock_guard<std::mutex> lk(up.mu); up.done = true; }
        up.cv.notify_one();
        up.th.join();
        lap("wait for the level uploads");
        if (st >= 0) st = up.status;
        {
            const int last = (int)h->H.L.size() - 1;
            std::lock_guard<std::mutex> lk(h->sched_mu);
            for (auto& J : h->sched_jobs)
                if (J && J->level >= last) {
                    if (J->th.joinable()) J->th.join();
                    if (J->uploaded) J->S.release();
                    J.reset();
                }
        }
        if (st < 0) { h->L.resize(h->H.L.size()); fasp_hip_amg_destroy(h); return st; }
        h->param = *amgparam;
    } else {
        st = fasp_hip_amg_create_host(&h, A, amgparam);
        if (st < 0) return st;
        lap("host setup");
    }
    try { st = upload_hierarchy(h); }
    catch (const std::bad_alloc&) { std::printf("### ERROR: fasp_hip: host allocation failed during the upload\n"); st = ERROR_ALLOC_MEM; }
    lap("upload_hierarchy");
    if (st < 0) { fasp_hip_amg_destroy(h); return st; }
    *out = h;
    return FASP_SUCCESS;
}

void fasp_hip_amg_destroy(fasp_hip_amg* h)
{
    FASP_ENTRY();
    if (h) sched_jobs_join(h);
    if (!h) return;
    if (g_ctx.ready) (void)hipStreamSynchronize(g_ctx.stream);
    for (auto& D : h->L) free_level(D);
    double* v[] = {h->b, h->u, h->p, h->t, h->r, h->cp, h->cr, h->ct, h->cbest};
    for (double* q : v)
        if (q) (void)hipFree(q);
    if (h->d_lazy) (void)hipFree(h->d_lazy);
    if (h->reg_img) (void)hipFree(h->reg_img);
    if (h->h_lazy) (void)hipHostFree(h->h_lazy);
    for (auto& e : h->ev) { (void)hipEventDestroy(e.a); (void)hipEventDestroy(e.b); }
    if (h->spcg_state) (void)hipFree(h->spcg_state);
    if (h->spcg_fused_buf) (void)hipFree(h->spcg_fused_buf);
    {
        auto& P = h->persist;
        void* q[] = {P.vals, P.cols, P.wrow, P.wend, P.t2, P.sync};
        for (void* x : q) if (x) (void)hipFree(x);
    }
    ShmMapping map{nullptr, 0};
    for (size_t q = 0; q < g_attached.size(); ++q)
        if (g_attached[q].first == h) { map = g_attached[q].second; g_attached.erase(g_attached.begin() + (long)q); break; }
    delete h;
    if (map.base) munmap(map.base, map.bytes);
}

int fasp_hip_coding_selftest(const dCSRmat* A, int* kind_out)
{
    FASP_ENTRY();
    if (!A || !kind_out) return ERROR_INPUT_PAR;
    HostCSR M;
    M.row = A->row; M.col = A->col; M.nnz = A->nnz;
    M.ia.alloc((size_t)A->row + 1); M.ja.alloc((size_t)std::max(A->nnz, 1)); M.val.alloc((size_t)std::max(A->nnz, 1));
    std::memcpy(M.ia.data(), A->IA, sizeof(int) * ((size_t)A->row + 1));
    std::memcpy(M.ja.data(), A->JA, sizeof(int) * (size_t)A->nnz);
    std::memcpy(M.val.data(), A->val, sizeof(double) * (size_t)A->nnz);
    const bool square = M.row == M.col;
    *kind_out = 0;
    if (!(M.nnz >= 4096 && (double)M.nnz <= 48.0 * M.row)) return FASP_SUCCESS;
    auto bits = [](double v) { unsigned long long b; std::memcpy(&b, &v, 8); return b; };
    {
        Buf<unsigned short> pat; Buf<int> rb;
        std::vector<int> pstart, plen, poff; std::vector<double> pval;
        if (build_rowpat(M, pat, pstart, plen, poff, pval, rb)) {
            *kind_out = 5;
            for (int r = 0; r < M.row; ++r) {
                const int id = pat[r], base = square ? r : rb[r];
                if (plen[id] != M.ia[r + 1] - M.ia[r]) return ERROR_MISC;
                for (int j = 0; j < plen[id]; ++j) {
                    const int k = M.ia[r] + j;
                    if (base + poff[pstart[id] + j] != M.ja[k] || bits(pval[pstart[id] + j]) != bits(M.val[k])) return ERROR_MISC;
                }
                for (int j = plen[id]; j < (plen[id] + 7) / 8 * 8; ++j)
                    if (poff[pstart[id] + j] != 0 || bits(pval[pstart[id] + j]) != 0ull) return ERROR_MISC;
            }
            return FASP_SUCCESS;
        }
    }
    {
        std::vector<int> doff; std::vector<double> dval;
        Buf<unsigned char> code; Buf<int> rb;
        if (build_dict8(M, doff, dval, code, rb)) {
            *kind_out = 4;
            for (int r = 0; r < M.row; ++r) {
                const int base = square ? r : rb[r];
                for (int k = M.ia[r]; k < M.ia[r + 1]; ++k)
                    if (base + doff[code[k]] != M.ja[k] || bits(dval[code[k]]) != bits(M.val[k])) return ERROR_MISC;
            }
        }
    }
    return FASP_SUCCESS;
}

int fasp_hip_amg_num_levels(const fasp_hip_amg* h) { return h ? (int)h->H.L.size() : ERROR_INPUT_PAR; }

int fasp_hip_amg_kernel_info(const fasp_hip_amg* h, int level, int which, int* kind, double* matrix_bytes)
{
    FASP_ENTRY();
    if (!h || level < 0 || level >= (int)h->L.size() || which < 0 || which > 2) return ERROR_INPUT_PAR;
    const DevLevel& D = h->L[level];
    const DevCSR& M = which == 0 ? D.A : which == 1 ? D.P : D.R;
    if (!M.ia) return ERROR_INPUT_PAR;
    double bytes = 0.0;
    const int k = kernel_family(M, &bytes);
    if (kind) *kind = k;
    if (matrix_bytes) *matrix_bytes = bytes;
    return FASP_SUCCESS;
}

int fasp_hip_coarse_kernel_info(const fasp_hip_amg* h, int* info)
{
    FASP_ENTRY();
    if (!h || !info) return ERROR_INPUT_PAR;
    for (int i = 0; i < 6; ++i) info[i] = h->coarse_kinfo[i];
    info[6] = g_ctx.num_cu; info[7] = 0;
    return FASP_SUCCESS;
}

int fasp_hip_bsr_coarse_kernel_info(const fasp_hip_amg_bsr* h, int* info)
{
    FASP_ENTRY();
    if (!h || !info) return ERROR_INPUT_PAR;
    for (int i = 0; i < 6; ++i) info[i] = h->coarse_kinfo[i];
    info[6] = g_ctx.num_cu; info[7] = 0;
    return FASP_SUCCESS;
}

int fasp_hip_amg_get_matrix(const fasp_hip_amg* h, int level, int which, dCSRmat* view)
{
    FASP_ENTRY();
    if (!h || !view || level < 0 || level >= (int)h->H.L.size()) return ERROR_INPUT_PAR;
    const HostLevel& L = h->H.L[level];
    if (which != 0 && !L.has_coarse) return ERROR_INPUT_PAR;
    *view = which == 0 ? L.A.view() : which == 1 ? L.P.view() : L.R.view();
    return FASP_SUCCESS;
}

int fasp_hip_amg_get_cfmark(const fasp_hip_amg* h, int level, ivector* view)
{
    FASP_ENTRY();
    if (!h || !view || level < 0 || level >= (int)h->H.L.size() || !h->H.L[level].has_coarse)
        return ERROR_INPUT_PAR;
    view->row = h->H.L[level].A.row;
    view->val = const_cast<int*>(h->H.L[level].cfmark.data());
    return FASP_SUCCESS;
}

int fasp_hip_set_rhs(fasp_hip_amg* h, const dvector* b)
{
    FASP_ENTRY();
    if (!h || !b || h->L.empty()) return ERROR_INPUT_PAR;
    const DevLevel& D0 = h->L[0];
    if (b->row != D0.nglobal) return ERROR_MAT_SIZE;
    HIPCK(hipMemcpyAsync(h->b, b->val + D0.row0, sizeof(double) * D0.nloc, hipMemcpyHostToDevice, g_ctx.stream));
    HIPCK(hipStreamSynchronize(g_ctx.stream));
    return FASP_SUCCESS;
}

int fasp_hip_set_guess(fasp_hip_amg* h, const dvector* x)
{
    FASP_ENTRY();
    if (!h || h->L.empty()) return ERROR_INPUT_PAR;
    const DevLevel& D0 = h->L[0];
    if (x) {
        if (x->row != D0.nglobal) return ERROR_MAT_SIZE;
        HIPCK(hipMemcpyAsync(h->u, x->val + D0.row0, sizeof(double) * D0.nloc, hipMemcpyHostToDevice, g_ctx.stream));
    } else {
        HIPCK(hipMemsetAsync(h->u, 0, sizeof(double) * D0.nvec, g_ctx.stream));
    }
    HIPCK(hipStreamSynchronize(g_ctx.stream));
    return FASP_SUCCESS;
}

int fasp_hip_get_solution(fasp_hip_amg* h, dvector* x)
{
    FASP_ENTRY();
    if (!h || !x || h->L.empty()) return ERROR_INPUT_PAR;
    const DevLevel& D0 = h->L[0];
    if (x->row != D0.nglobal) return ERROR_MAT_SIZE;
    HIPCK(hipMemcpyAsync(x->val + D0.row0, h->u, sizeof(double) * D0.nloc, hipMemcpyDeviceToHost, g_ctx.stream));
    HIPCK(hipStreamSynchronize(g_ctx.stream));
    return FASP_SUCCESS;
}

int fasp_hip_device_synchronize(void)
{
    FASP_ENTRY();
    if (!g_ctx.ready) return FASP_SUCCESS;
    HIPCK(hipStreamSynchronize(g_ctx.stream));
    return FASP_SUCCESS;
}

int fasp_hip_solve_resident(fasp_hip_amg* h, const ITS_param* itparam, double* hist, int hist_cap,
                            fasp_hip_stats* stats)
{
    FASP_ENTRY();
    if (!h || !itparam) return ERROR_INPUT_PAR;
    if (h->L.empty()) return ERROR_INPUT_PAR;
    int st = check_supported(itparam, &h->param);
    if (st < 0) return st;
    its_check(itparam->tol, itparam->maxit);

    h->ev_used = 0;
    h->use_fmg = itparam->precond_type == PREC_FMG;
    const long long ci0 = h->coarse_iters, vc0 = h->vcycles;
    Hist   H{hist, hist_cap, 0};
    PcgOut po{BIGREAL, BIGREAL, BIGREAL};
    const double t0 = wall_seconds();
    {
        KOps K = csr_ops(h, 0, true);
        const KParams P{itparam->tol, itparam->abstol, itparam->maxit, (short)itparam->restart, itparam->stop_type, itparam->print_level};
        st = krylov_run(K, (KMethod)itparam->itsolver_type, K_OFFER_ALL, false, P, h->b, h->u, h->p, h->t, h->r, &H, &po);
    }
    HIPCK(hipStreamSynchronize(g_ctx.stream));
    if (seq_err_check() < 0) return ERROR_MISC;
    const double t_solve = wall_seconds() - t0;

    if (stats) {
        stats->iters = st; stats->nhist = H.n; stats->relres = po.relres; stats->absres = po.absres;
        stats->normr0 = po.normr0; stats->solve_seconds = t_solve; stats->upload_seconds = 0.0;
        double ms = 0.0;
        for (int i = 0; i < h->ev_used; ++i) {
            float e = 0.f;
            if (hipEventElapsedTime(&e, h->ev[i].a, h->ev[i].b) == hipSuccess) ms += e;
        }
        stats->spmv_launches = h->ev_used;
        stats->spmv_ms = h->ev_used ? ms / h->ev_used : 0.0;
        stats->coarse_iters = h->coarse_iters - ci0;
        stats->vcycles = h->vcycles - vc0;
    }
    print_itsolver_time(itparam->print_level, st, t_solve);
    return st;
}

int fasp_hip_solve(fasp_hip_amg* h, const dvector* b, dvector* x, const ITS_param* itparam, double* hist,
                   int hist_cap, fasp_hip_stats* stats)
{
    FASP_ENTRY();
    if (!h || !b || !x || !itparam) return ERROR_INPUT_PAR;
    double t0 = wall_seconds();
    int st = fasp_hip_set_rhs(h, b);
    if (st < 0) return st;
    if ((st = fasp_hip_set_guess(h, x)) < 0) return st;
    double t_up = wall_seconds() - t0;
    st = fasp_hip_solve_resident(h, itparam, hist, hist_cap, stats);
    t0 = wall_seconds();
    const int st2 = fasp_hip_get_solution(h, x);
    if (st2 < 0) return st2;
    t_up += wall_seconds() - t0;
    if (stats) stats->upload_seconds = t_up;
    return st;
}

int fasp_hip_amg_solve(fasp_hip_amg* h, const dvector* b, dvector* x, const AMG_param* param, double* hist,
                       int hist_cap, fasp_hip_stats* stats)
{
    FASP_ENTRY();
    if (!h || !b || !x || h->L.empty()) return ERROR_INPUT_PAR;
    const AMG_param& p = param ? *param : h->param;
    int st = check_supported(nullptr, &p);
    if (st < 0) return st;
    double t0 = wall_seconds();
    if ((st = fasp_hip_set_rhs(h, b)) < 0) return st;
    if ((st = fasp_hip_set_guess(h, x)) < 0) return st;
    double t_up = wall_seconds() - t0;
    h->ev_used = 0;
    const long long ci0 = h->coarse_iters, vc0 = h->vcycles;
    Hist   H{hist, hist_cap, 0};
    PcgOut po{BIGREAL, BIGREAL, BIGREAL};
// ... 1182 lines not shown
    const size_t n = (size_t)A->ROW * A->nb;
    TmpVec du(u->val, n), dun(nullptr, n), db(b->val, n), dd(diaginv, (size_t)A->ROW * A->nb * A->nb);
    BsrArgs a{}; a.x = du.d; a.y = dun.d; a.b = db.d; a.dinv = dd.d;
    launch_bsr<2>(M, a);
    dun.get(u->val);
}

int fasp_hip_bsr_sweep(const dBSRmat* A, const double* b, double* u, const double* diaginv, int descend, int sor, double w,
                       int* nlevels)
{
    FASP_ENTRY();
    if (!A || !b || !u || !diaginv || !nlevels || !A->IA || (A->NNZ > 0 && (!A->JA || !A->val))) return ERROR_INPUT_PAR;
    if (A->nb < 1 || A->nb > 7 || A->storage_manner != 0 || A->ROW != A->COL || A->ROW < 0 || A->NNZ < 0) return ERROR_INPUT_PAR;
    TmpBSR M(A);
    if (!M.ok) return ERROR_MISC;
    const size_t n = (size_t)A->ROW * A->nb;
    TmpVec du(u, n), db(b, n), dd(diaginv, n * A->nb);
    if (!du.d || !db.d || !dd.d) return ERROR_MISC;
    DevLevel::Sched S;
    int st = bsr_seq_schedule(A->ROW, A->COL, A->NNZ, A->IA, A->JA, descend != 0, S);
    if (st >= 0) st = bsr_seq_launch(M, S, db.d, dd.d, du.d, sor != 0, w);
    if (st >= 0) { *nlevels = (int)S.ptr.size() - 1; du.get(u); }
    else (void)hipStreamSynchronize(g_ctx.stream);
    S.release();
    return st;
}

double fasp_hip_time_bsr_mxv(const dBSRmat* A, int reps)
{
    FASP_ENTRY();
    TmpBSR M(A);
    if (!M.ok || reps <= 0) return -1.0;
    TmpVec dx(nullptr, (size_t)A->COL * A->nb), dy(nullptr, (size_t)A->ROW * A->nb);
    (void)hipMemsetAsync(dx.d, 0, sizeof(double) * dx.n, g_ctx.stream);
    BsrArgs a{}; a.x = dx.d; a.y = dy.d;
    hipEvent_t e0, e1;
    (void)hipEventCreate(&e0); (void)hipEventCreate(&e1);
    launch_bsr<0>(M, a); launch_bsr<0>(M, a);
    (void)hipEventRecord(e0, g_ctx.stream);
    for (int i = 0; i < reps; ++i) launch_bsr<0>(M, a);
    (void)hipEventRecord(e1, g_ctx.stream);
    (void)hipEventSynchronize(e1);
    float ms = 0.f;
    (void)hipEventElapsedTime(&ms, e0, e1);
    (void)hipEventDestroy(e0); (void)hipEventDestroy(e1);
    return (double)ms / reps;
}

void fasp_smoother_dcsr_jacobi(dvector* u, const int i_1, const int i_n, const int s, dCSRmat* A, dvector* b,
                               int L, const double w)
{
    FASP_ENTRY();
    (void)s;
    TmpCSR M(A);
    if (!M.ok) die_no_device(__func__);
    const int n = A->row;
    const int lo = std::min(i_1, i_n), hi = std::max(i_1, i_n);
    if (lo != 0 || hi != n - 1) {
        std::fprintf(stderr, "### ERROR: fasp_smoother_dcsr_jacobi (device): only full sweeps 0..n-1 supported\n");
        std::exit(ERROR_INPUT_PAR);
    }
    std::vector<double> d(n, 0.0);
    bool dup = false;
    for (int i = 0; i < n; ++i) {
        int hits = 0;
        for (int k = A->IA[i]; k < A->IA[i + 1]; ++k)
            if (A->JA[k] == i) { d[i] = A->val[k]; ++hits; }
        dup = dup || hits > 1;
    }
    M.D.dup_diag = dup;
    TmpVec du(u->val, n), du2(nullptr, n), db(b->val, n), dd(d.data(), n);
    double *x = du.d, *xo = du2.d;
    while (L--) {
        CsrArgs a{};
        a.x = x; a.y = xo; a.b = db.d; a.diag = dd.d; a.omega = w;
        launch_csr<OP_JACOBI>(M.D, a);
        std::swap(x, xo);
    }
    (void)hipStreamSynchronize(g_ctx.stream);
    (void)hipMemcpy(u->val, x, sizeof(double) * n, hipMemcpyDeviceToHost);
}

#ifdef FLOW_TIMING
extern "C" int fasp_hip_flow_times(unsigned long long* out, int n)
{
    FASP_ENTRY();
    return hipMemcpyFromSymbol(out, HIP_SYMBOL(fasp::g_flow_times), sizeof(unsigned long long) * (size_t)std::min(n, 8192)) == hipSuccess ? 0 : -1;
}
#endif

static int g_time_cold = 0;
int fasp_hip_tune(const char* key, int value)
{
    FASP_ENTRY();
    if (!key) return ERROR_INPUT_PAR;
    if (!std::strcmp(key, "maxgrid")) g_tune.maxgrid = value;
    else if (!std::strcmp(key, "xcd")) g_tune.xcd = value;
    else if (!std::strcmp(key, "gen2")) g_tune.gen2 = value;
    else if (!std::strcmp(key, "ws2_bpc")) g_tune.ws2_bpc = value;
    else if (!std::strcmp(key, "nt")) g_tune.nt = value;
    else if (!std::strcmp(key, "kind")) g_tune.kind = value;
    else if (!std::strcmp(key, "compress")) g_tune.compress = value;
    else if (!std::strcmp(key, "rpl")) g_tune.rpl = value;
    else if (!std::strcmp(key, "lds_tab")) g_tune.lds_tab = value;
    else if (!std::strcmp(key, "xcd_pat")) g_tune.xcd_pat = value;
    else if (!std::strcmp(key, "spcg_batch")) g_tune.spcg_batch = value;
    else if (!std::strcmp(key, "spcg_fused")) g_tune.spcg_fused = value;
    else if (!std::strcmp(key, "spcg_persist")) { g_tune.spcg_persist = value; if (value) g_persist_disabled = false; }
    else if (!std::strcmp(key, "spcg_test_hang")) g_tune.spcg_test_hang = value;
    else if (!std::strcmp(key, "spcg_grid")) g_tune.spcg_grid = value;
    else if (!std::strcmp(key, "small_lds")) g_tune.small_lds = value;
    else if (!std::strcmp(key, "small_onewave")) g_tune.small_onewave = value;
    else if (!std::strcmp(key, "ja16")) g_tune.ja16 = value;
    else if (!std::strcmp(key, "device_sort")) g_device_sort = value;
    else if (!std::strcmp(key, "halo_overlap")) g_halo_overlap = value;
    else if (!std::strcmp(key, "coarse_mode")) g_coarse_mode = value;
    else if (!std::strcmp(key, "coarse_split_min")) g_coarse_split_min = value;
    else if (!std::strcmp(key, "split_rows")) g_tune.split_rows = value;
    else if (!std::strcmp(key, "gs_multicolor")) g_tune.gs_multicolor = value;
    else if (!std::strcmp(key, "seq_flow")) { g_tune.seq_flow = value; if (value) g_flow_disabled = false; }
    else if (!std::strcmp(key, "ilu_smooth_fused")) g_tune.ilu_smooth_fused = value;
    else if (!std::strcmp(key, "ilu_form")) g_tune.ilu_form = value;
    else if (!std::strcmp(key, "seq_strip_kb")) g_tune.seq_strip_kb = value;
    else if (!std::strcmp(key, "seq_jobs")) g_tune.seq_jobs = value;
    else if (!std::strcmp(key, "local_square")) g_tune.local_square = value;
    else if (!std::strcmp(key, "seq_grid")) g_tune.seq_grid = value;
    else if (!std::strcmp(key, "seq_chain")) g_tune.seq_chain = value;
    else if (!std::strcmp(key, "seq_chain_n1")) g_tune.seq_chain_n1 = value;
    else if (!std::strcmp(key, "seq_chain_grid")) g_tune.seq_chain_grid = value;
    else if (!std::strcmp(key, "seq_test_hang")) g_tune.seq_test_hang = value;
    else if (!std::strcmp(key, "seq_rest_lanes")) g_tune.seq_rest_lanes = value;
    else if (!std::strcmp(key, "seq_chain_ref")) g_tune.seq_chain_ref = value;
    else if (!std::strcmp(key, "seq_spine")) g_tune.seq_spine = value;
    else if (!std::strcmp(key, "seq_partition")) g_seq_partition = value;
    else if (!std::strcmp(key, "fuse_zr")) g_tune.fuse_zr = value;
    else if (!std::strcmp(key, "fuse_presmooth")) g_tune.fuse_presmooth = value;
    else if (!std::strcmp(key, "seq_lanes")) g_tune.seq_lanes = value;
    else if (!std::strcmp(key, "lazy_coarse")) g_tune.lazy_coarse = value;
    else if (!std::strcmp(key, "xtile")) g_tune.xtile = value;
    else if (!std::strcmp(key, "rp5_max")) g_tune.rp5_max = value;
    else if (!std::strcmp(key, "rp_bpc")) g_tune.rp_bpc = value;
    else if (!std::strcmp(key, "rp_stream")) g_tune.rp_stream = value;
    else if (!std::strcmp(key, "renumber")) g_tune.renumber = value;
    else if (!std::strcmp(key, "renumber_chunk")) g_tune.renumber_chunk = value;
    else if (!std::strcmp(key, "time_cold")) g_time_cold = value;
    else if (!std::strcmp(key, "estream")) g_tune.estream = value;
    else if (!std::strcmp(key, "sell")) g_tune.sell = value;
    else if (!std::strcmp(key, "es_dbg")) g_tune.es_dbg = value;
    else if (!std::strcmp(key, "pcg_dev_beta")) g_tune.pcg_dev_beta = value;
    else if (!std::strcmp(key, "seq_chain_touch")) g_tune.seq_chain_touch = value;
    else if (!std::strcmp(key, "seq_chain_touch_t1")) g_tune.seq_chain_touch_t1 = value;
    else if (!std::strcmp(key, "seq_zero_skip")) g_tune.seq_zero_skip = value;
    else if (!std::strcmp(key, "pcg_fold")) g_tune.pcg_fold = value;
    else if (!std::strcmp(key, "spcg_spec")) g_tune.spcg_spec = value;
    else if (!std::strcmp(key, "ev_every")) g_tune.ev_every = value;
    else if (!std::strcmp(key, "rp_xcd")) g_tune.rp_xcd = value;
    else if (!std::strcmp(key, "rp_strip")) g_tune.rp_strip = value;
    else if (!std::strcmp(key, "host_parallel_min")) g_parallel_min_nnz = value;
    else if (!std::strcmp(key, "rap_form")) g_rap_form = value;
    else if (!std::strcmp(key, "rap_arena_kb")) g_rap_arena_kb = value;
    else if (!std::strcmp(key, "device_rap")) g_device_rap = value;
    else if (!std::strcmp(key, "lanes")) g_tune.lanes = value;
    else if (!std::strcmp(key, "wrows")) g_tune.wrows = value;
    else if (!std::strcmp(key, "wcap")) g_tune.wcap = value;
    else return ERROR_INPUT_PAR;
    return FASP_SUCCESS;
}

int fasp_hip_sell_selftest(const dCSRmat* A, int cap_percent, int* info, double* bytes, int* ia_out, int* ja_out, double* val_out, const double* x, double* y)
{
    if (!A || !info || A->row < 0 || A->nnz < 0) return ERROR_INPUT_PAR;
    HostCSR M;
    M.row = A->row; M.col = A->col; M.nnz = A->nnz;
    M.ia.view(A->IA, (size_t)A->row + 1); M.ja.view(A->JA, (size_t)std::max(A->nnz, 1)); M.val.view(A->val, (size_t)std::max(A->nnz, 1));
    SellHost S;
    int why = 0;
    const bool ok = build_sell(M, S, cap_percent > 0 ? cap_percent : SELL_CAP_PERCENT, &why);
    info[0] = ok ? 1 : 0; info[1] = why; info[2] = S.nv; info[3] = S.vbits; info[4] = S.obits; info[5] = S.nslice;
    info[6] = ok ? (int)std::min<long long>(S.slots / 64, 0x7fffffff) : 0; info[7] = SELL_MAXV;
    if (bytes) *bytes = ok ? S.bytes(M.row) : 0.0;
    if (!ok) return FASP_SUCCESS;
    if (ia_out && ja_out && val_out) sell_decode_host(S, M.row, ia_out, ja_out, val_out);
    if (x && y) sell_mxv_host(S, M.row, x, y);
    return FASP_SUCCESS;
}

int fasp_hip_csr_plan(const int* traits, int op, int windowed, int want_partials, int* plan, double* bytes)
{
    FASP_ENTRY();
    if (!traits || !plan || op < OP_MXV || op > OP_MXV_DOT) return ERROR_INPUT_PAR;
    static double dummy[1];
    const int* t = traits;
    auto flag = [&](int i) -> void* { return t[i] ? dummy : nullptr; };
    DevCSR M;
    M.row = t[0]; M.col = t[1]; M.nnz = t[2]; M.kind = t[3]; M.lanes = t[4]; M.wrows = t[5]; M.wcap = t[6]; M.nxrows = t[7]; M.plane = t[8];
    M.npat = t[9]; M.npent = t[10]; M.sell_nv = t[11]; M.sell_nslice = t[12]; M.sell_slots = t[13]; M.ntcols = t[14]; M.es_W = t[15]; M.es_nc = t[16];
    M.code = (unsigned char*)flag(17); M.pat = (unsigned short*)flag(18); M.rowbase = (int*)flag(19); M.dpos = (int*)flag(20); M.dup_diag = t[21] != 0;
    M.ja16 = (unsigned short*)flag(22); M.jbase = (int*)flag(23); M.lja16 = (unsigned short*)flag(24); M.sell_code = (unsigned*)flag(25);
    M.es_tab = (int*)flag(26); M.es_ja16 = (unsigned short*)flag(27);
    const CsrPlan p = plan_csr(M, op, windowed || g_tune.split_rows > 0, want_partials != 0);
    const int out[11] = {(int)p.kernel, p.family, p.tile_rows, p.bpc, p.xcd_map, p.tpp, p.nt, p.ja16, p.jbase, p.fused_zr, kernel_family(M, nullptr)};
    std::copy(out, out + 11, plan);
    if (bytes) *bytes = p.bytes;
    return FASP_SUCCESS;
}

int fasp_hip_estream_selftest(const int* ia, int nrow, int nnz, int per_wave, int wmax, int* info)
{
    if (!ia || nrow < 1 || nnz < 1 || per_wave < 8 || wmax < 32) return ERROR_INPUT_PAR;
    return estream_selftest_host(ia, nrow, nnz, per_wave, wmax, info);
}

int fasp_hip_measure_ceilings(double* out, size_t bytes, int reps)
{
    FASP_ENTRY();
    if (!out || bytes < (1u << 20) || reps <= 0) return ERROR_INPUT_PAR;
    if (ctx_init() != FASP_SUCCESS) return ERROR_MISC;
    f64x2_t *p = nullptr, *q = nullptr, *r = nullptr;
    HIPCK(hipMalloc(&p, bytes)); HIPCK(hipMalloc(&q, bytes)); HIPCK(hipMalloc(&r, bytes));
    HIPCK(hipMemsetAsync(p, 0, bytes, g_ctx.stream)); HIPCK(hipMemsetAsync(q, 0, bytes, g_ctx.stream));
    HIPCK(hipMemsetAsync(r, 0, bytes, g_ctx.stream));
    const size_t n16 = bytes / 16;
    hipEvent_t e0, e1;
    HIPCK(hipEventCreate(&e0)); HIPCK(hipEventCreate(&e1));
    const int grid = 4 * g_ctx.num_cu;
    for (int which = 0; which < 3; ++which) {
        auto run = [&]() {
            if (which == 0) hipLaunchKernelGGL(k_read16, dim3(grid), dim3(BLOCK), 0, g_ctx.stream, n16, p, (double*)q);
            else if (which == 1) hipLaunchKernelGGL(k_copy16, dim3(grid), dim3(BLOCK), 0, g_ctx.stream, n16, p, q);
            else hipLaunchKernelGGL(k_triad16, dim3(grid), dim3(BLOCK), 0, g_ctx.stream, n16, 0.5, p, q, r);
        };
        run(); run();
        HIPCK(hipEventRecord(e0, g_ctx.stream));
        for (int i = 0; i < reps; ++i) run();
        HIPCK(hipEventRecord(e1, g_ctx.stream));
        HIPCK(hipEventSynchronize(e1));
        float ms = 0.f;
        HIPCK(hipEventElapsedTime(&ms, e0, e1));
        out[which] = (double)(which + 1) * (double)bytes * reps / ((double)ms * 1e-3) / 1e9;
    }
    (void)hipEventDestroy(e0); (void)hipEventDestroy(e1);
    (void)hipFree(p); (void)hipFree(q); (void)hipFree(r);
    return FASP_SUCCESS;
}

double fasp_hip_time_kernel(fasp_hip_amg* h, int kind, int level, int reps)
{
    FASP_ENTRY();
    if (!h || level < 0 || level >= (int)h->L.size() || reps <= 0) return -1.0;
    DevLevel& D = h->L[level];
    const int n = D.A.row;
    hipEvent_t e0, e1;
    if (hipEventCreate(&e0) != hipSuccess || hipEventCreate(&e1) != hipSuccess) return -1.0;
    double* x = D.xa; double* y = D.xb; double* w = D.w;
    auto run = [&]() {
        switch (kind) {
            case 0: d_mxv(D.A, x, y); break;
            case 1: d_aAxpy(-1.0, D.A, x, y); break;
            case 2: { CsrArgs a{}; a.x = x; a.y = y; a.b = w; a.diag = D.diag; a.omega = 0.6667; launch_csr<OP_JACOBI>(D.A, a); } break;
            case 3: hipLaunchKernelGGL(k_dot, dim3(vec_grid(n)), dim3(BLOCK), 0, g_ctx.stream, n, x, y, g_ctx.d_partials); break;
            case 4: d_axpy(n, 0.5, x, y); break;
            case 5: { CsrArgs a{}; a.x = x; a.y = y; a.dotv = x; a.partials = g_ctx.d_partials; launch_csr<OP_MXV_DOT>(D.A, a); } break;
            case 6: if (D.R.ia) d_mxv(D.R, w, h->L[level + 1].xa); break;
            case 7: if (D.P.ia) d_aAxpy(1.0, D.P, h->L[level + 1].xa, y); break;
            case 8:
                if (D.A.val) hipLaunchKernelGGL(k_read16, dim3(2048), dim3(BLOCK), 0, g_ctx.stream, (size_t)D.A.nnz / 2, (const f64x2_t*)D.A.val, y);
                break;
            case 10: case 11: case 12: case 13: (void)seq_sweep(h, level, kind - 10, 1, 1.0); break;
            default: break;
        }
    };
    (void)hipMemsetAsync(x, 0, sizeof(double) * n, g_ctx.stream);
    (void)hipMemsetAsync(y, 0, sizeof(double) * n, g_ctx.stream);
    (void)hipMemsetAsync(w, 0, sizeof(double) * n, g_ctx.stream);
    double* const keep_b = D.b; double* const keep_x = D.x;
    if (kind >= 10) { D.b = w; D.x = x; }
    if (g_time_cold) {
        double* big = nullptr;
        const size_t bigb = (size_t)512 << 20;
        if (hipMalloc(&big, bigb + 4096) != hipSuccess) return -1.0;
        (void)hipMemsetAsync(big, 0, bigb, g_ctx.stream);
        double tot = 0.0;
        for (int i = 0; i < reps + 1; ++i) {
            if (g_time_cold >= 2) (void)hipMemsetAsync(big, 0, bigb, g_ctx.stream);
            else hipLaunchKernelGGL(k_read16, dim3(1024), dim3(BLOCK), 0, g_ctx.stream, bigb / 16, (const f64x2_t*)big, big + bigb / 8);
            (void)hipEventRecord(e0, g_ctx.stream);
            run();
            (void)hipEventRecord(e1, g_ctx.stream);
            (void)hipEventSynchronize(e1);
            float ms1 = 0.f;
            (void)hipEventElapsedTime(&ms1, e0, e1);
            if (i >= 1) tot += ms1;
        }
        (void)hipFree(big);
        D.b = keep_b; D.x = keep_x;
        (void)hipEventDestroy(e0); (void)hipEventDestroy(e1);
        return tot / reps;
    }
    run(); run();
    (void)hipEventRecord(e0, g_ctx.stream);
    for (int i = 0; i < reps; ++i) run();
    (void)hipEventRecord(e1, g_ctx.stream);
    (void)hipEventSynchronize(e1);
    D.b = keep_b; D.x = keep_x;
    float ms = 0.f;
    (void)hipEventElapsedTime(&ms, e0, e1);
// ... 128 lines not shown
```

include/fasp_hip_dev.h:

```cpp
#ifndef FASP_HIP_DEV_H
#define FASP_HIP_DEV_H
#include "fasp_hip.h"
#ifdef __cplusplus
extern "C" {
#endif

double fasp_hip_time_kernel(fasp_hip_amg* h, int kind, int level, int reps);
double fasp_hip_time_matrix(const dCSRmat* A, int op, int reps, int* kind_out);
double fasp_hip_seq_schedule_selftest(const dCSRmat* A, const int* seq, int ns, int strip_kb, int lanes, int spine, int* info);
int fasp_hip_cluster_order(const dCSRmat* A, int chunk, int* order);
int fasp_hip_permute_csr(const dCSRmat* A, const int* rperm, const int* cinv, int* ia, int* ja, double* val);
double fasp_hip_seq_chain_selftest(const dCSRmat* A, const int* seq, int ns, int n1_blocks, int form, double w, int* info, double* out_u);
int fasp_hip_measure_ceilings(double* out, size_t bytes, int reps);

int    fasp_hip_ilu_resident_count(void);
double fasp_hip_ilu_time(ILU_data* iludata, int which, int reps, double* info);
int    fasp_hip_bsr_amg_get_ilu(const fasp_hip_amg_bsr* h, int level, ILU_data* view);
int    fasp_hip_bsr_amg_ilu_info(const fasp_hip_amg_bsr* h, int level, double info[6]);
double fasp_hip_bsr_amg_ilu_smooth_time(fasp_hip_amg_bsr* h, int level, int reps);

int    fasp_hip_dcsr_rap(const dCSRmat* R, const dCSRmat* A, const dCSRmat* P, dCSRmat* RAP);
int    fasp_hip_rap_info(int info[4]);
long   fasp_hip_rap_device_count(void);
double fasp_hip_rap_time(const dCSRmat* R, const dCSRmat* A, const dCSRmat* P, int where, int reps);

int fasp_hip_tune(const char* key, int value);
int fasp_hip_coarse_kernel_info(const fasp_hip_amg* h, int* info);
int fasp_hip_bsr_coarse_kernel_info(const fasp_hip_amg_bsr* h, int* info);

int fasp_hip_comm_stats(double* out8, int reset);
int fasp_hip_comm_timing(int on);

int fasp_hip_dist_plan(fasp_hip_amg* h, int rank, int nranks, int min_rows);
int fasp_hip_dist_level_info(const fasp_hip_amg* h, int level, int* info);
int fasp_hip_dist_get_matrix(const fasp_hip_amg* h, int level, int which, dCSRmat* view);
int fasp_hip_dist_get_list(const fasp_hip_amg* h, int level, int which, ivector* view);
int  fasp_hip_estream_selftest(const int* ia, int nrow, int nnz, int per_wave, int wmax, int* info);
int  fasp_hip_csr_plan(const int* traits, int op, int windowed, int want_partials, int* plan, double* bytes);
int  fasp_hip_sell_selftest(const dCSRmat* A, int cap_percent, int* info, double* bytes, int* ia_out, int* ja_out, double* val_out, const double* x, double* y);
int  fasp_hip_level_op(fasp_hip_amg* h, int level, int which, int op, const double* x, const double* b, double* y, double* y2, double scalar, double* red);
int  fasp_hip_matrix_op(const dCSRmat* A, int op, const double* x, const double* b, double* y, double* y2, double scalar, double* red, int* kind_out);
int  fasp_hip_bsr_sweep(const dBSRmat* A, const double* b, double* u, const double* diaginv, int descend, int sor, double w, int* nlevels);
int  fasp_hip_comm_selftest(void);

#ifdef __cplusplus
}
#endif
#endif
```

Baseline: 483.0 million.

## Fold coarse PCG setup and convergence check into persistent kernel

The persistent coarse-grid PCG kernel now does its own startup: it loads the initial residual, zeroes the solution and computes the initial norm, so the separate init launch is skipped. When the kernel detects convergence it publishes u across blocks, has the worker blocks compute A*u, and the lead block forms the true residual b-Au and its norm. The host then reads this tail record instead of launching a separate residual and dot-product check. This removes several launches and host round-trips per coarse solve, at the cost of an extra cross-block exchange epoch, a larger scratch buffer and more complex hang and epoch bookkeeping.

```diff
diff --git a/faspsolver_amd/__init__.py b/faspsolver_amd/__init__.py
--- a/faspsolver_amd/__init__.py
+++ b/faspsolver_amd/__init__.py
@@ -20,7 +20,7 @@
     "fasp_solver_dbsr_pcg", "fasp_solver_dbsr_pbcgs", "fasp_solver_dbsr_pgmres", "fasp_solver_dbsr_pvgmres",
     "fasp_solver_dbsr_pvfgmres", "fasp_hip_bsr_precond_setup", "fasp_hip_bsr_precond_fct", "fasp_hip_bsr_precond_free",
     "fasp_hip_param_input", "fasp_fwrapper_dcsr_krylov_amg_", "fasp_dcsrvec_read2", "fasp_dvec_read",
-    "fasp_dbsr_read", "fasp_dcoo_read", "fasp_dcoo_read1", "fasp_dcoo_shift_read", "fasp_dmtx_read", "fasp_dmtxsym_read", "fasp_dvec_write", "fasp_dcsr_write_coo", "fasp_dcsrvec_write2", "fasp_fwrapper_dcsr_amg_", "fasp_fwrapper_dbsr_krylov_amg_", "fasp_hip_free_bsr", "fasp_hip_comm_selftest", "fasp_hip_amg_kernel_info", "fasp_hip_coarse_kernel_info", "fasp_hip_bsr_coarse_kernel_info", "fasp_hip_coding_selftest", "fasp_solver_amg", "fasp_solver_famg", "fasp_hip_amg_solve", "fasp_precond_diag", "fasp_precond_dbsr_diag", "fasp_solver_dcsr_itsolver", "fasp_solver_dcsr_krylov", "fasp_solver_dcsr_krylov_diag", "fasp_solver_dbsr_itsolver", "fasp_solver_dbsr_krylov", "fasp_solver_dbsr_krylov_diag", "fasp_hip_mxv_csr", "fasp_hip_mxv_bsr", "fasp_solver_matfree_init", "fasp_solver_pcg", "fasp_solver_pbcgs", "fasp_solver_pgcg", "fasp_solver_pminres", "fasp_solver_pgmres", "fasp_solver_pvgmres", "fasp_solver_pvfgmres", "fasp_solver_itsolver", "fasp_solver_krylov", "fasp_solver_dcsr_pcg", "fasp_solver_dcsr_pminres", "fasp_solver_dcsr_pgcg", "fasp_solver_dcsr_pgcr", "fasp_solver_dcsr_pbcgs", "fasp_solver_dcsr_pgmres", "fasp_solver_dcsr_pvgmres",
+    "fasp_dbsr_read", "fasp_dcoo_read", "fasp_dcoo_read1", "fasp_dcoo_shift_read", "fasp_dmtx_read", "fasp_dmtxsym_read", "fasp_dvec_write", "fasp_dcsr_write_coo", "fasp_dcsrvec_write2", "fasp_fwrapper_dcsr_amg_", "fasp_fwrapper_dbsr_krylov_amg_", "fasp_hip_free_bsr", "fasp_hip_comm_selftest", "fasp_hip_amg_kernel_info", "fasp_hip_coarse_kernel_info", "fasp_hip_coarse_handback", "fasp_hip_bsr_coarse_kernel_info", "fasp_hip_coding_selftest", "fasp_solver_amg", "fasp_solver_famg", "fasp_hip_amg_solve", "fasp_precond_diag", "fasp_precond_dbsr_diag", "fasp_solver_dcsr_itsolver", "fasp_solver_dcsr_krylov", "fasp_solver_dcsr_krylov_diag", "fasp_solver_dbsr_itsolver", "fasp_solver_dbsr_krylov", "fasp_solver_dbsr_krylov_diag", "fasp_hip_mxv_csr", "fasp_hip_mxv_bsr", "fasp_solver_matfree_init", "fasp_solver_pcg", "fasp_solver_pbcgs", "fasp_solver_pgcg", "fasp_solver_pminres", "fasp_solver_pgmres", "fasp_solver_pvgmres", "fasp_solver_pvfgmres", "fasp_solver_itsolver", "fasp_solver_krylov", "fasp_solver_dcsr_pcg", "fasp_solver_dcsr_pminres", "fasp_solver_dcsr_pgcg", "fasp_solver_dcsr_pgcr", "fasp_solver_dcsr_pbcgs", "fasp_solver_dcsr_pgmres", "fasp_solver_dcsr_pvgmres",
     "fasp_solver_dcsr_pvfgmres", "fasp_hip_precond_setup", "fasp_hip_precond_fct", "fasp_hip_precond_free",
     "fasp_hip_time_bsr_mxv", "fasp_solver_dbsr_krylov_amg", "fasp_hip_bsr_amg_create", "fasp_hip_bsr_amg_create_host",
     "fasp_hip_bsr_amg_destroy", "fasp_hip_bsr_amg_num_levels", "fasp_hip_bsr_amg_get_matrix",
diff --git a/faspsolver_amd/csrc/coarse_cg.hip.h b/faspsolver_amd/csrc/coarse_cg.hip.h
--- a/faspsolver_amd/csrc/coarse_cg.hip.h
+++ b/faspsolver_amd/csrc/coarse_cg.hip.h
@@ -73,12 +73,12 @@
     }
     bool ok = hipMalloc(&P.vals, tot * sizeof(double)) == hipSuccess && hipMalloc(&P.cols, tot * sizeof(unsigned short)) == hipSuccess &&
               hipMalloc(&P.wrow, sizeof(int) * (size_t)nw * 8) == hipSuccess && hipMalloc(&P.wend, sizeof(int) * (size_t)nw * 8) == hipSuccess &&
-              hipMalloc(&P.t2, sizeof(double) * 4 * (size_t)m) == hipSuccess && hipMalloc(&P.sync, 1024) == hipSuccess;
+              hipMalloc(&P.t2, sizeof(double) * 6 * (size_t)m) == hipSuccess && hipMalloc(&P.sync, 1024) == hipSuccess;
     if (ok) ok = hipMemcpy(P.vals, vals.data(), tot * sizeof(double), hipMemcpyHostToDevice) == hipSuccess &&
                  hipMemcpy(P.cols, cols.data(), tot * sizeof(unsigned short), hipMemcpyHostToDevice) == hipSuccess &&
                  hipMemcpy(P.wrow, wrow.data(), sizeof(int) * (size_t)nw * 8, hipMemcpyHostToDevice) == hipSuccess &&
                  hipMemcpy(P.wend, wend.data(), sizeof(int) * (size_t)nw * 8, hipMemcpyHostToDevice) == hipSuccess;
-    if (ok) ok = hipMemset(P.t2, 0, sizeof(double) * 4 * (size_t)m) == hipSuccess;
+    if (ok) ok = hipMemset(P.t2, 0, sizeof(double) * 6 * (size_t)m) == hipSuccess && hipMemset(P.sync, 0, 1024) == hipSuccess;
     if (!ok) return false;
     P.NE = NE; P.nblocks = nblocks; P.ok = true;
     return true;
@@ -214,7 +214,21 @@
     const bool fused = g_tune.spcg_fused && m <= 8000 && A.val && A.ja && !A.code && !A.pat;
     bool persist = fused && g_tune.spcg_persist && !g_persist_disabled && !comm_shares_devices() &&
                    (size_t)m * 24 <= 150 * 1024 && build_persist_plan(h, (int)(&D - &h->L[0]));
-    if (!h->spcg_state) HIPCK(hipMalloc(&h->spcg_state, sizeof(SpcgState)));
+    static_assert(sizeof(SpcgState) % 8 == 0 && sizeof(SpcgState) + sizeof(SpcgTail) + 24 <= sizeof(double) * 64, "the state, its tail, the error word and the speculative norm fit the pinned scratch");
+    if (!h->spcg_state) {
+        HIPCK(hipMalloc(&h->spcg_state, sizeof(SpcgState) + sizeof(SpcgTail)));
+        HIPCK(hipMemset(h->spcg_state, 0, sizeof(SpcgState) + sizeof(SpcgTail)));
+    }
+    SpcgTail* const d_tail = reinterpret_cast<SpcgTail*>(h->spcg_state + 1);
+    const bool tail = persist && g_tune.spcg_tail != 0;
+    bool tail_start = tail, tail_forced = false;
+    const bool x_zero_start = D.x_zero;
+    if (g_tune.spcg_tail == 2) { h->handback_r.clear(); h->handback_u.clear(); }
+    if (tail) {
+        if (!D.x_zero) d_resid(A, u, b, r);
+        D.x_zero = false;
+        goto ITERATE;
+    }
     if (fused) {
         if (!D.x_zero) d_resid(A, u, b, r);
         SpcgInitArgs ia{};
@@ -267,13 +281,27 @@
             if (persist) {
                 auto& PP = h->persist;
                 PP.launches = (PP.launches + 1u) & 0x1fffffu;
-                if (PP.launches == 0u) { HIPCK(hipMemsetAsync(PP.t2, 0, sizeof(double) * 4 * (size_t)m, s)); PP.launches = 1u; }
+                if (PP.launches == 0u) {
+                    HIPCK(hipMemsetAsync(PP.t2, 0, sizeof(double) * 6 * (size_t)m, s));
+                    HIPCK(hipMemsetAsync(PP.sync, 0, 1024, s));
+                    HIPCK(hipMemsetAsync(&d_tail->err, 0, sizeof(unsigned), s));
+                    PP.launches = 1u;
+                }
                 SpcgPersistArgs pa{};
                 pa.epoch0 = PP.launches << 11;
                 pa.m = m; pa.max_steps = MaxIt + 2; pa.nblocks = PP.nblocks; pa.st = h->spcg_state;
                 pa.r = r; pa.p = p; pa.u = u; pa.u_best = u_best; pa.t2 = PP.t2; pa.sync = PP.sync;
                 pa.vals = PP.vals; pa.cols = PP.cols; pa.wrow = PP.wrow; pa.wend = PP.wend;
-                HIPCK(hipMemsetAsync(PP.sync, 0, 1024, s));
+                if (tail) {
+                    pa.err = &d_tail->err; pa.err_tag = PP.launches;
+                    pa.start = tail_start ? 1 : 0; pa.x_zero = x_zero_start ? 1 : 0;
+                    pa.tail = (g_tune.spcg_tail == 2 && !tail_forced) ? 2 : 1;
+                    pa.MaxIt = MaxIt; pa.tol = tol; pa.maxdiff = maxdiff; pa.b = b; pa.tl = d_tail;
+                    tail_start = false;
+                } else {
+                    pa.err = PP.sync + 3; pa.err_tag = 1u;
+                    HIPCK(hipMemsetAsync(PP.sync, 0, 1024, s));
+                }
                 pa.u_lds = (sizeof(double) * 4 * (size_t)m + 1024 <= 160 * 1024) ? 1 : 0;
                 const size_t lds = sizeof(double) * (pa.u_lds ? 4 : 3) * (size_t)m;
                 int lst;
@@ -311,20 +339,25 @@
                 h->coarse_kinfo[0] = 7; h->coarse_kinfo[1] = m <= 512 * 4 ? 4 : m <= 512 * 10 ? 10 : 0; h->coarse_kinfo[2] = 0;
             }
             bool spec_rr = false;
-            if (persist && g_tune.spcg_spec) {
+            if (persist && !tail && g_tune.spcg_spec) {
                 d_resid(A, u, b, t);
                 if (d_dot_to(m, t, t, 14, false) < 0) return ERROR_MISC;
                 spec_rr = true;
             }
-            HIPCK(hipMemcpyAsync(g_ctx.h_part, h->spcg_state, sizeof(SpcgState), hipMemcpyDeviceToHost, s));
-            static_assert(sizeof(SpcgState) % 8 == 0 && sizeof(SpcgState) + 24 <= sizeof(double) * 64, "the error word and the speculative norm travel behind the state");
-            if (persist) HIPCK(hipMemcpyAsync(reinterpret_cast<char*>(g_ctx.h_part) + sizeof(SpcgState), h->persist.sync, 16, hipMemcpyDeviceToHost, s));
+            const bool tail_now = persist && tail;
+            HIPCK(hipMemcpyAsync(g_ctx.h_part, h->spcg_state, sizeof(SpcgState) + (tail_now ? sizeof(SpcgTail) : 0), hipMemcpyDeviceToHost, s));
+            if (persist && !tail) HIPCK(hipMemcpyAsync(reinterpret_cast<char*>(g_ctx.h_part) + sizeof(SpcgState), h->persist.sync, 16, hipMemcpyDeviceToHost, s));
             if (spec_rr) HIPCK(hipMemcpyAsync(reinterpret_cast<char*>(g_ctx.h_part) + sizeof(SpcgState) + 16, g_ctx.d_red + 14, 8, hipMemcpyDeviceToHost, s));
             HIPCK(hipStreamSynchronize(s));
             std::memcpy(&S, g_ctx.h_part, sizeof(S));
             double spec_val = 0.0;
             if (spec_rr) std::memcpy(&spec_val, reinterpret_cast<char*>(g_ctx.h_part) + sizeof(SpcgState) + 16, 8);
-            if (persist) {
+            SpcgTail T{};
+            if (tail_now) {
+                std::memcpy(&T, reinterpret_cast<char*>(g_ctx.h_part) + sizeof(SpcgState), sizeof(T));
+                if (T.err == h->persist.launches && S.stop == SPCG_RUN) S.stop = SPCG_HANG;
+                if (S.stop != SPCG_CONV) T.check3 = 0u;
+            } else if (persist) {
                 unsigned ew[4];
                 std::memcpy(ew, reinterpret_cast<char*>(g_ctx.h_part) + sizeof(SpcgState), 16);
                 if (ew[3] != 0u && S.stop == SPCG_RUN) S.stop = SPCG_HANG;
@@ -381,7 +414,16 @@
                 ++stag;
             }
             if (relres < tol) {
-                if (spec_rr && S.stop != SPCG_HANG) red[0] = spec_val;
+                if (T.check3) {
+                    red[0] = T.rr;
+                    if (T.check3 == 2u && g_tune.spcg_tail == 2 && !tail_forced) {
+                        tail_forced = true;
+                        h->handback_r.resize((size_t)m); h->handback_u.resize((size_t)m);
+                        HIPCK(hipMemcpy(h->handback_r.data(), r, sizeof(double) * m, hipMemcpyDeviceToHost));
+                        HIPCK(hipMemcpy(h->handback_u.data(), u, sizeof(double) * m, hipMemcpyDeviceToHost));
+                    }
+                }
+                else if (spec_rr && S.stop != SPCG_HANG) red[0] = spec_val;
                 else {
                     spec_rr = false;
                     d_resid(A, u, b, r);
@@ -389,7 +431,8 @@
                 }
                 absres = std::sqrt(red[0]);
                 relres = absres / normr0;
-                if (relres < tol) break;
+                if (T.check3) { absres = T.absres; relres = T.relres; }
+                if (T.check3 ? T.check3 == 1u : relres < tol) break;
                 if (spec_rr) HIPCK(hipMemcpyAsync(r, t, sizeof(double) * m, hipMemcpyDeviceToDevice, s));
                 if (more_step >= MAX_RESTART) { iter = ERROR_SOLVER_TOLSMALL; break; }
                 HIPCK(hipMemsetAsync(p, 0, sizeof(double) * m, s));
diff --git a/faspsolver_amd/csrc/device_csr.hip.h b/faspsolver_amd/csrc/device_csr.hip.h
--- a/faspsolver_amd/csrc/device_csr.hip.h
+++ b/faspsolver_amd/csrc/device_csr.hip.h
@@ -1005,7 +1005,7 @@
     return build_estream(H.ia.data(), H.row, H.nnz, D);
 }
 
-struct Tuning { int ilu_smooth_fused = 1, gen2 = 2, ws2_bpc = 3, maxgrid = -1, xcd = 16, nt = 1, kind = -1, lanes = -1, wrows = -1, wcap = -1, compress = 1, rpl = -1, lds_tab = 1, xcd_pat = 64, spcg_batch = 16, small_lds = 1, ja16 = 1, spcg_fused = 1, spcg_grid = 0, spcg_persist = 1, split_rows = 0, gs_multicolor = 0, seq_flow = 1, seq_strip_kb = 0, seq_jobs = 1, seq_spine = 1, seq_grid = 0, seq_chain = 1, seq_chain_n1 = 0, seq_chain_grid = 0, seq_chain_ref = 0, seq_test_hang = 0, seq_rest_lanes = 0, local_square = 1, fuse_zr = 1, fuse_presmooth = 1, seq_lanes = 0, xtile = 1, rp5_max = 45, rp_bpc = 5, rp_xcd = -1, rp_strip = 2, spcg_test_hang = 0, small_onewave = 4, lazy_coarse = 1, rp_stream = -1, renumber = 1, renumber_chunk = 262144, pcg_dev_beta = 1, spcg_spec = 1, ev_every = 4, pcg_fold = 1, seq_chain_touch = 8, seq_chain_touch_t1 = 1, seq_zero_skip = 1, estream = 1, es_dbg = 0, ilu_form = -1, sell = 1; };
+struct Tuning { int ilu_smooth_fused = 1, gen2 = 2, ws2_bpc = 3, maxgrid = -1, xcd = 16, nt = 1, kind = -1, lanes = -1, wrows = -1, wcap = -1, compress = 1, rpl = -1, lds_tab = 1, xcd_pat = 64, spcg_batch = 16, small_lds = 1, ja16 = 1, spcg_fused = 1, spcg_grid = 0, spcg_persist = 1, split_rows = 0, gs_multicolor = 0, seq_flow = 1, seq_strip_kb = 0, seq_jobs = 1, seq_spine = 1, seq_grid = 0, seq_chain = 1, seq_chain_n1 = 0, seq_chain_grid = 0, seq_chain_ref = 0, seq_test_hang = 0, seq_rest_lanes = 0, local_square = 1, fuse_zr = 1, fuse_presmooth = 1, seq_lanes = 0, xtile = 1, rp5_max = 45, rp_bpc = 5, rp_xcd = -1, rp_strip = 2, spcg_test_hang = 0, small_onewave = 4, lazy_coarse = 1, rp_stream = -1, renumber = 1, renumber_chunk = 262144, pcg_dev_beta = 1, spcg_spec = 1, ev_every = 4, pcg_fold = 1, seq_chain_touch = 8, seq_chain_touch_t1 = 1, seq_zero_skip = 1, estream = 1, es_dbg = 0, ilu_form = -1, sell = 1, spcg_tail = 1; };
 static Tuning g_tune;
 
 template <class K>
diff --git a/faspsolver_amd/csrc/hierarchy.hip.h b/faspsolver_amd/csrc/hierarchy.hip.h
--- a/faspsolver_amd/csrc/hierarchy.hip.h
+++ b/faspsolver_amd/csrc/hierarchy.hip.h
@@ -81,6 +81,7 @@
     double*              spcg_fused_buf = nullptr;
     int                  spcg_last_iters = 0;
     SpcgState*           spcg_state = nullptr;
+    std::vector<double>  handback_r, handback_u;
     struct Persist { bool tried = false, ok = false; int NE = 0, nblocks = 0; double* vals = nullptr; unsigned short* cols = nullptr;
                      int *wrow = nullptr, *wend = nullptr; double* t2 = nullptr; unsigned* sync = nullptr; unsigned launches = 0; } persist;
     std::vector<double>  amli_coef;
diff --git a/faspsolver_amd/csrc/small_solvers.hip.h b/faspsolver_amd/csrc/small_solvers.hip.h
--- a/faspsolver_amd/csrc/small_solvers.hip.h
+++ b/faspsolver_amd/csrc/small_solvers.hip.h
@@ -1776,6 +1776,11 @@
 #define SPCG_POLL_GROUP 6
 #endif
 
+struct SpcgTail {
+    unsigned err;
+    unsigned check3;
+    double   rr, absres, relres;
+};
 struct SpcgPersistArgs {
     int        m, max_steps, nblocks;
     int        u_lds;
@@ -1788,6 +1793,15 @@
     const unsigned short* cols;
     const int*            wrow;
     const int*            wend;
+    unsigned*             err;
+    unsigned              err_tag;
+    int           start;
+    int           x_zero;
+    int           tail;
+    int           MaxIt;
+    double        tol, maxdiff;
+    const double* b;
+    SpcgTail*     tl;
 };
 
 __device__ __forceinline__ void lds_barrier()
@@ -1836,12 +1850,41 @@
     double* sr = dyn + m;
     double* st = dyn + 2 * m;
     double* su = dyn + 3 * m;
-    gu32* g_err = (gu32*)(a.sync + 3);
+    gu32* g_err = (gu32*)a.err;
     gu64* g_verdict = (gu64*)(a.sync + 8);
     __shared__ int s_hang;
     typedef unsigned int pu32x4 __attribute__((ext_vector_type(4)));
     SpcgState& S = *a.st;
-    if (S.stop != SPCG_RUN) return;
+    const bool start = a.start != 0, u_lds = a.u_lds != 0;
+    if (!start && S.stop != SPCG_RUN) return;
+
+    double temp1, best, normr0, tol, maxdiff;
+    int    it0, stag, MaxIt, iter_best;
+    double o_tp, o_rr, o_uu, o_pp, o_maxu, o_nan, o_alpha, o_absres, o_relres, o_temp1_prev;
+    int steps_done = 0, my_stop = SPCG_RUN, stop0 = SPCG_RUN;
+    if (start) {
+        const bool xz = a.x_zero != 0;
+        double v0[1] = {0.0};
+        for (int i = tid; i < m; i += NT) {
+            const double ri = xz ? a.b[i] : a.r[i];
+            sp[i] = ri; sr[i] = ri;
+            if (lead) {
+                a.u_best[i] = 0.0;
+                if (xz) { if (u_lds) su[i] = 0.0; else a.u[i] = 0.0; }
+                else if (u_lds) su[i] = a.u[i];
+            }
+            v0[0] += ri * ri;
+        }
+        blk_reduce_dpp<1, NW>(v0, sh);
+        const double absres0 = sqrt(v0[0]);
+        normr0 = fmax(1e-20, absres0);
+        temp1 = v0[0]; best = 1e+20; tol = a.tol; maxdiff = a.maxdiff;
+        it0 = 0; stag = 1; MaxIt = a.MaxIt; iter_best = 0;
+        o_tp = 0.0; o_rr = v0[0]; o_uu = 0.0; o_pp = 0.0; o_maxu = 0.0; o_nan = 0.0; o_alpha = 0.0;
+        o_absres = 1e+20; o_relres = absres0 / normr0; o_temp1_prev = v0[0];
+        if (o_relres < tol) stop0 = SPCG_ZERO_RHS;
+        if (lead) my_stop = stop0;
+    }
 
     double   v[NE];
     unsigned cpk[NE / 2];
@@ -1859,21 +1902,19 @@
         if (lane < 8) { endsv = a.wend[gw * 8 + lane]; rowsv = a.wrow[gw * 8 + lane]; }
         my_rows = __popcll(__ballot(lane < 8 && rowsv >= 0));
     }
-    for (int i = tid; i < m; i += NT) { sp[i] = a.p[i]; sr[i] = a.r[i]; }
-    const bool u_lds = a.u_lds != 0;
-    if (lead && u_lds) for (int i = tid; i < m; i += NT) su[i] = a.u[i];
-    double temp1 = S.temp1;
-    const double absres_best0 = S.absres_best, normr0 = S.normr0, tol = S.tol, maxdiff = S.maxdiff;
-    const int    it0 = S.iter, stag = S.stag, MaxIt = S.MaxIt;
-    double best = absres_best0;
-    int    iter_best = S.iter_best;
-    double o_tp = S.tp, o_rr = S.rr, o_uu = S.uu, o_pp = S.pp, o_maxu = S.maxu, o_nan = S.nan, o_alpha = S.alpha,
-           o_absres = S.absres, o_relres = S.relres, o_temp1_prev = S.temp1_prev;
-    int steps_done = 0, my_stop = SPCG_RUN;
+    if (!start) {
+        for (int i = tid; i < m; i += NT) { sp[i] = a.p[i]; sr[i] = a.r[i]; }
+        if (lead && u_lds) for (int i = tid; i < m; i += NT) su[i] = a.u[i];
+        temp1 = S.temp1; best = S.absres_best; normr0 = S.normr0; tol = S.tol; maxdiff = S.maxdiff;
+        it0 = S.iter; stag = S.stag; MaxIt = S.MaxIt; iter_best = S.iter_best;
+        o_tp = S.tp; o_rr = S.rr; o_uu = S.uu; o_pp = S.pp; o_maxu = S.maxu; o_nan = S.nan; o_alpha = S.alpha;
+        o_absres = S.absres; o_relres = S.relres; o_temp1_prev = S.temp1_prev;
+    }
+    const double temp1_in = temp1;
     if (tid == 0) {
         s_hang = 0;
         if (lead)
-            __hip_atomic_store(g_verdict, ((unsigned long long)(a.epoch0 + 1u) << 32) | (unsigned)SPCG_RUN, __ATOMIC_RELAXED, __HIP_MEMORY_SCOPE_AGENT);
+            __hip_atomic_store(g_verdict, ((unsigned long long)(a.epoch0 + 1u) << 32) | (unsigned)stop0, __ATOMIC_RELAXED, __HIP_MEMORY_SCOPE_AGENT);
     }
     __syncthreads();
 #ifdef SPCG_PERSIST_STAMPS
@@ -1882,12 +1923,44 @@
 #else
 #define STAMP(q) do { } while (0)
 #endif
-
-    for (int step = 0; step < a.max_steps; ++step) {
+    auto poll = [&](const __amdgpu_buffer_rsrc_t rs, const unsigned epq, double* dst, const unsigned long long t0) -> bool {
+        bool hung = false;
+#pragma unroll 1
+        for (int e0 = 0; e0 < E && !hung; e0 += SPCG_POLL_GROUP) {
+#ifdef SPCG_PERSIST_STAMPS
+            if (e0 == 6 && !LEAD) STAMP(6);
+#endif
+            unsigned pend = 0u;
+#pragma unroll
+            for (int e = 0; e < SPCG_POLL_GROUP; ++e) if (tid + (e0 + e) * NT < m) pend |= 1u << e;
+            while (pend) {
+#ifdef SPCG_PERSIST_STAMPS
+                tk[7] += 1;
+#endif
+                pu32x4 q[SPCG_POLL_GROUP];
+#pragma unroll
+                for (int e = 0; e < SPCG_POLL_GROUP; ++e)
+                    q[e] = __builtin_amdgcn_raw_buffer_load_b128(rs, ((pend >> e) & 1u) ? (tid + (e0 + e) * NT) * 16 : (int)0xfffffff0u, 0, 16 );
+#pragma unroll
+                for (int e = 0; e < SPCG_POLL_GROUP; ++e)
+                    if (((pend >> e) & 1u) && q[e].y == epq && q[e].w == epq) {
+                        dst[tid + (e0 + e) * NT] = __longlong_as_double((long long)(((unsigned long long)q[e].z << 32) | q[e].x));
+                        pend &= ~(1u << e);
+                    }
+                if (pend && __builtin_amdgcn_s_memrealtime() - t0 > 200000000ull) { hung = true; break; }
+            }
+        }
+        return hung;
+    };
+
+    int      epi = 0;
+    unsigned chk3 = 0u;
+    double   t_rr = 0.0, t_absres = 0.0, t_relres = 0.0;
+    for (int step = 0; step < a.max_steps || epi; ++step) {
         const int par = step & 1;
         const unsigned ep = a.epoch0 + (unsigned)step + 1u;
         const __amdgpu_buffer_rsrc_t tr =
-            __builtin_amdgcn_make_buffer_rsrc(a.t2 + (size_t)par * 2 * m, 0, (int)((unsigned)m * 16u), 0x00020000);
+            __builtin_amdgcn_make_buffer_rsrc(a.t2 + (size_t)(epi ? 2 : par) * 2 * m, 0, (int)((unsigned)m * 16u), 0x00020000);
         if (!lead && my_rows > 0 && my_stop == SPCG_RUN) {
             double acc = 0.0;
             int    j = 0;
@@ -1913,38 +1986,14 @@
                 }
             }
         }
+        if (epi && !lead) break;
         STAMP(0);
         {
             const unsigned long long t0 = __builtin_amdgcn_s_memrealtime();
-            bool hung = false;
             unsigned long long vr0 = 0ull;
-            if (tid == 0) vr0 = __hip_atomic_load(g_verdict + par, __ATOMIC_RELAXED, __HIP_MEMORY_SCOPE_AGENT);
-#pragma unroll 1
-            for (int e0 = 0; e0 < E && !hung; e0 += SPCG_POLL_GROUP) {
-#ifdef SPCG_PERSIST_STAMPS
-                if (e0 == 6 && !LEAD) STAMP(6);
-#endif
-                unsigned pend = 0u;
-#pragma unroll
-                for (int e = 0; e < SPCG_POLL_GROUP; ++e) if (tid + (e0 + e) * NT < m) pend |= 1u << e;
-                while (pend) {
-#ifdef SPCG_PERSIST_STAMPS
-                    tk[7] += 1;
-#endif
-                    pu32x4 q[SPCG_POLL_GROUP];
-#pragma unroll
-                    for (int e = 0; e < SPCG_POLL_GROUP; ++e)
-                        q[e] = __builtin_amdgcn_raw_buffer_load_b128(tr, ((pend >> e) & 1u) ? (tid + (e0 + e) * NT) * 16 : (int)0xfffffff0u, 0, 16 );
-#pragma unroll
-                    for (int e = 0; e < SPCG_POLL_GROUP; ++e)
-                        if (((pend >> e) & 1u) && q[e].y == ep && q[e].w == ep) {
-                            st[tid + (e0 + e) * NT] = __longlong_as_double((long long)(((unsigned long long)q[e].z << 32) | q[e].x));
-                            pend &= ~(1u << e);
-                        }
-                    if (pend && __builtin_amdgcn_s_memrealtime() - t0 > 200000000ull) { hung = true; break; }
-                }
-            }
-            if (tid == 0 && !hung) {
+            if (tid == 0 && !epi) vr0 = __hip_atomic_load(g_verdict + par, __ATOMIC_RELAXED, __HIP_MEMORY_SCOPE_AGENT);
+            bool hung = poll(tr, ep, st, t0);
+            if (tid == 0 && !hung && !epi) {
                 int flag = -1;
                 for (bool first = true;; first = false) {
                     const unsigned long long vr = first ? vr0 : __hip_atomic_load(g_verdict + par, __ATOMIC_RELAXED, __HIP_MEMORY_SCOPE_AGENT);
@@ -1956,13 +2005,34 @@
             }
             if (hung) {
                 s_hang = 1;
-                __hip_atomic_store(g_err, 1u, __ATOMIC_RELAXED, __HIP_MEMORY_SCOPE_AGENT);
+                __hip_atomic_store(g_err, a.err_tag, __ATOMIC_RELAXED, __HIP_MEMORY_SCOPE_AGENT);
             }
         }
         lds_barrier();
         STAMP(1);
         if (s_hang) { my_stop = SPCG_HANG; break; }
+        if (epi) break;
         const int flag = s_flag;
+        if (flag == SPCG_CONV && a.tail) {
+            const __amdgpu_buffer_rsrc_t ur =
+                __builtin_amdgcn_make_buffer_rsrc(a.t2 + (size_t)(par ^ 1) * 2 * m, 0, (int)((unsigned)m * 16u), 0x00020000);
+            const unsigned epu = ep + 1u;
+            if (lead) {
+                for (int i = tid; i < m; i += NT) {
+                    const unsigned long long bits = (unsigned long long)__double_as_longlong(u_lds ? su[i] : a.u[i]);
+                    const pu32x4 rec = {(unsigned)bits, epu, (unsigned)(bits >> 32), epu};
+                    __builtin_amdgcn_raw_buffer_store_b128(rec, ur, i * 16, 0, 16 );
+                }
+            } else if (poll(ur, epu, sp, __builtin_amdgcn_s_memrealtime())) {
+                s_hang = 1;
+                __hip_atomic_store(g_err, a.err_tag, __ATOMIC_RELAXED, __HIP_MEMORY_SCOPE_AGENT);
+            }
+            lds_barrier();
+            if (s_hang) { my_stop = SPCG_HANG; break; }
+            epi = 1;
+            ++step;
+            continue;
+        }
         if (flag != SPCG_RUN) break;
         if (my_stop != SPCG_RUN) break;
         STAMP(2);
@@ -2086,14 +2156,27 @@
 #undef STAMP
 
     if (lead) {
-        for (int i = tid; i < m; i += NT) { a.r[i] = sr[i]; a.p[i] = sp[i]; if (u_lds) a.u[i] = su[i]; }
+        if (epi && my_stop != SPCG_HANG) {
+            double v3[1] = {0.0};
+            for (int i = tid; i < m; i += NT) {
+                const double rt = a.b[i] - st[i];
+                st[i] = rt;
+                v3[0] += rt * rt;
+            }
+            blk_reduce_dpp<1, NW>(v3, sh);
+            t_rr = v3[0]; t_absres = sqrt(t_rr); t_relres = t_absres / normr0;
+            chk3 = (t_relres < tol && a.tail != 2) ? 1u : 2u;
+        }
+        for (int i = tid; i < m; i += NT) { a.r[i] = (chk3 == 2u) ? st[i] : sr[i]; a.p[i] = sp[i]; if (u_lds) a.u[i] = su[i]; }
         if (tid == 0) {
             S.tp = o_tp; S.rr = o_rr; S.uu = o_uu; S.pp = o_pp; S.maxu = o_maxu; S.nan = o_nan;
             S.alpha = o_alpha; S.absres = o_absres; S.relres = o_relres;
             S.absres_best = best; S.iter_best = iter_best; S.iter = it0 + steps_done;
             S.temp1_prev = o_temp1_prev;
-            S.temp1 = (my_stop == SPCG_DIV0) ? S.temp1 : temp1;
+            S.temp1 = (my_stop == SPCG_DIV0) ? temp1_in : temp1;
             S.stop = my_stop;
+            if (start) { S.normr0 = normr0; S.tol = tol; S.maxdiff = maxdiff; S.stag = stag; S.MaxIt = MaxIt; S.pad = 0; }
+            if (a.tl) { a.tl->check3 = chk3; a.tl->rr = t_rr; a.tl->absres = t_absres; a.tl->relres = t_relres; }
         }
     }
 }
diff --git a/faspsolver_amd/csrc/solver.hip b/faspsolver_amd/csrc/solver.hip
--- a/faspsolver_amd/csrc/solver.hip
+++ b/faspsolver_amd/csrc/solver.hip
@@ -535,6 +535,17 @@
     for (int i = 0; i < 6; ++i) info[i] = h->coarse_kinfo[i];
     info[6] = g_ctx.num_cu; info[7] = 0;
     return FASP_SUCCESS;
+}
+
+int fasp_hip_coarse_handback(const fasp_hip_amg* h, double* r, double* u, int n)
+{
+    FASP_ENTRY();
+    if (!h || !r || !u) return ERROR_INPUT_PAR;
+    const size_t m = h->handback_r.size();
+    if (m == 0 || (size_t)n < m) return 0;
+    std::memcpy(r, h->handback_r.data(), sizeof(double) * m);
+    std::memcpy(u, h->handback_u.data(), sizeof(double) * m);
+    return (int)m;
 }
 
 int fasp_hip_bsr_coarse_kernel_info(const fasp_hip_amg_bsr* h, int* info)
@@ -2023,6 +2034,7 @@
     else if (!std::strcmp(key, "seq_chain_touch_t1")) g_tune.seq_chain_touch_t1 = value;
     else if (!std::strcmp(key, "seq_zero_skip")) g_tune.seq_zero_skip = value;
     else if (!std::strcmp(key, "pcg_fold")) g_tune.pcg_fold = value;
+    else if (!std::strcmp(key, "spcg_tail")) g_tune.spcg_tail = value;
     else if (!std::strcmp(key, "spcg_spec")) g_tune.spcg_spec = value;
     else if (!std::strcmp(key, "ev_every")) g_tune.ev_every = value;
     else if (!std::strcmp(key, "rp_xcd")) g_tune.rp_xcd = value;
diff --git a/include/fasp_hip_dev.h b/include/fasp_hip_dev.h
--- a/include/fasp_hip_dev.h
+++ b/include/fasp_hip_dev.h
@@ -26,6 +26,7 @@
 
 int fasp_hip_tune(const char* key, int value);
 int fasp_hip_coarse_kernel_info(const fasp_hip_amg* h, int* info);
+int fasp_hip_coarse_handback(const fasp_hip_amg* h, double* r, double* u, int n);
 int fasp_hip_bsr_coarse_kernel_info(const fasp_hip_amg_bsr* h, int* info);
 
 int fasp_hip_comm_stats(double* out8, int reset);
```

Result: no change. 486.2 million (median of 6 runs) (+0.7%).
